# silencht/SG-SLAM

Measured on AMD Instinct MI355X. Metric: tracked frames/sec (640x480 RGB-D), higher is better.
Workload: dtype u8/f32(bf16x3 matrix products)/f64

## Files before the change

include/sgx_debug.h:

```cpp
#ifndef SGX_DEBUG_H
#define SGX_DEBUG_H
#include "sgx.h"
#ifdef __cplusplus
extern "C" {
#endif

int sgx_orb_debug_level_geometry(const sgx_orb *h, int level, int32_t *w, int32_t *hgt, int32_t *stride);
int sgx_orb_debug_set_unfused_pyramid(int on);
int sgx_orb_debug_read_level(sgx_orb *h, int frame, int level, uint8_t *dst );
int sgx_orb_debug_read_candidates(sgx_orb *h, int frame, int level, int32_t *x, int32_t *y, int32_t *score, int cap, int *n);
int sgx_debug_flow_affine_batch_dev(int batch, int cap, const sgx_keypoint *d_keys, const int32_t *d_n, const float *d_A, const float *d_shift, const float *d_boxes,
                                    int max_boxes, float *d_prev_xy, void *stream);
int sgx_pose_opt_debug_set_threads(int threads_per_frame);
int sgx_ba_debug_last_plan(int32_t plan[4]);
int sgx_ba_debug_set_init(int mode);
int sgx_ba_debug_set_jobs(int host);
int sgx_ba_debug_set_solver(int mode);
int sgx_det_debug_read_blob(sgx_det *h, const char *blob_name, int image, float *dst, int cap, int *n);
int sgx_flow_debug_read_level(sgx_flow *h, int slot, int frame, int level, uint8_t *img);
int sgx_flow_debug_read_slot(sgx_flow *h, int slot, int frame, int level, uint8_t *img, int32_t *pitch);
int sgx_flow_debug_level_size(const sgx_flow *h, int level, int32_t *w, int32_t *hgt);
int sgx_pnp_debug_betas(int which, const double *L, const double *rho, double *betas);
int sgx_obj3d_debug_read(sgx_obj3d *h, int job, uint8_t *kept, int32_t *labels, int cap, int *n);
int sgx_cloud_debug_read(sgx_cloud *h, int image, sgx_cloud_point *voxels, float *dist, uint8_t *kept, int cap, int *n);
int sgx_debug_corun_bf16(int blocks, int iters, int launches, void *stream);
int sgx_det_debug_detection_output(sgx_det *h, const float *loc, const float *conf, int batch, sgx_det_result *results);
int sgx_det_debug_continued(sgx_det *h, int *count);
int sgx_det_debug_set_fusion(int on);
int sgx_det_debug_set_irb(int on);
int sgx_det_debug_set_block_fusion(int on);
int sgx_det_debug_set_gemm(int mode);
int sgx_det_debug_set_legacy_kernels(int on);
int sgx_det_debug_time_ops(sgx_det *h, const uint8_t *d_img, int pitch, int batch, int reps, float *ms, int cap, int *nops);
int sgx_det_debug_run_step(sgx_det *h, const uint8_t *d_img, int pitch, int batch, int step, int reps, void *stream);
int sgx_orb_debug_run_octree(sgx_orb *h, int level, const uint32_t *packed, int n, uint32_t *out_sel, int cap, int *nsel);
int sgx_orb_debug_read_plan(const sgx_orb *h, int section, void *dst, size_t cap, size_t *bytes);
int sgx_tracker_debug_set_describe_early(int on);
int sgx_tracker_debug_set_boxes(sgx_tracker *t, const float *boxes, const int32_t *nboxes, const int32_t *have_dynamic);
int sgx_tracker_debug_sync_trace(sgx_tracker *t, int32_t *dst, int cap, int *n);
int sgx_tracker_debug_fail_after(int n);
int sgx_debug_devmem_fail_after(int n);
int sgx_stereo_debug_read(sgx_stereo *h, int frame, int32_t *best_idx, int32_t *best_dist, int32_t *exit_code, int32_t *best_inc, int32_t *sads);

#ifdef __cplusplus
}
#endif
#endif
```

sg_slam_amd/capi.py:

```python
import ctypes as C
import numpy as np

KP_DTYPE = np.dtype([('x', 'f4'), ('y', 'f4'), ('size', 'f4'), ('angle', 'f4'), ('response', 'f4'),
                     ('octave', 'i4'), ('class_id', 'i4')])


class SgxError(RuntimeError):
    pass


class Camera(C.Structure):
    _fields_ = [('fx', C.c_float), ('fy', C.c_float), ('cx', C.c_float), ('cy', C.c_float), ('bf', C.c_float),
                ('min_x', C.c_float), ('max_x', C.c_float), ('min_y', C.c_float), ('max_y', C.c_float)]


class BaProblem(C.Structure):
    _fields_ = [('n_poses', C.c_int32), ('n_points', C.c_int32), ('n_edges', C.c_int32), ('poses', C.c_void_p), ('pose_fixed', C.c_void_p),
                ('points', C.c_void_p), ('edge_pose', C.c_void_p), ('edge_point', C.c_void_p), ('edge_obs', C.c_void_p), ('edge_info', C.c_void_p)]


class BaStats(C.Structure):
    _fields_ = [('iterations_first', C.c_int32), ('iterations_second', C.c_int32), ('free_poses', C.c_int32), ('reserved', C.c_int32),
                ('chi2_first', C.c_double), ('chi2_second', C.c_double)]


SGX_DET_MAX = 100


class Detection(C.Structure):
    _fields_ = [(k, C.c_float) for k in ('label', 'score', 'xmin', 'ymin', 'xmax', 'ymax')]


class Object2D(C.Structure):
    _fields_ = [('id', C.c_int32)] + [(k, C.c_float) for k in ('prob', 'x', 'y', 'w', 'h')]


class DetResult(C.Structure):
    _fields_ = [('n_raw', C.c_int32), ('raw', Detection * SGX_DET_MAX), ('n_objects', C.c_int32), ('objects', Object2D * SGX_DET_MAX),
                ('have_dynamic_for_mapping', C.c_int32), ('have_dynamic_for_rm_feature', C.c_int32),
                ('n_map_boxes', C.c_int32), ('map_boxes', Object2D * SGX_DET_MAX), ('n_rm_boxes', C.c_int32), ('rm_boxes', Object2D * SGX_DET_MAX)]


class FlowConfig(C.Structure):
    _fields_ = [('width', C.c_int32), ('height', C.c_int32), ('max_batch', C.c_int32), ('win_size', C.c_int32), ('max_level', C.c_int32),
                ('max_count', C.c_int32), ('epsilon', C.c_double)]


class TrackerConfig(C.Structure):
    _fields_ = [('streams', C.c_int32), ('width', C.c_int32), ('height', C.c_int32), ('nfeatures', C.c_int32), ('scale_factor', C.c_float), ('nlevels', C.c_int32),
                ('ini_th_fast', C.c_int32), ('min_th_fast', C.c_int32), ('cam', Camera), ('depth_map_factor', C.c_float), ('th_projection', C.c_float),
                ('local_map', C.c_int32), ('dynamic_mask', C.c_int32), ('max_boxes', C.c_int32), ('pipelined', C.c_int32)]


class Obj3dParams(C.Structure):
    _fields_ = [('sor_stddev_mul', C.c_double), ('sor_mean_k', C.c_int32), ('cluster_min_size', C.c_int32), ('cluster_max_size', C.c_int32),
                ('voxel_leaf_size', C.c_float), ('cluster_tolerance', C.c_float), ('similar_compare_ratio', C.c_float),
                ('camera_valid_depth_min', C.c_float), ('camera_valid_depth_max', C.c_float)]


class Obj3dJob(C.Structure):
    _fields_ = [('image', C.c_int32), ('class_id', C.c_int32)] + [(k, C.c_float) for k in ('prob', 'x', 'y', 'w', 'h')]


OBJ3D_RESULT_DTYPE = np.dtype([('found', 'i4'), ('class_id', 'i4'), ('prob', 'f4'), ('centroid', 'f4', 3), ('size', 'f4', 3), ('crop_points', 'i4'), ('kept_points', 'i4'),
                               ('components', 'i4'), ('clusters', 'i4'), ('best_cluster_size', 'i4'), ('larger_window_points', 'i4'), ('best_similar1', 'f4'),
                               ('best_similar2', 'f4'), ('best_roi', 'f4', 4)])


class SemanticObjectRecord(C.Structure):
    _fields_ = [('class_id', C.c_int32), ('object_id', C.c_int32), ('prob', C.c_float), ('centroid', C.c_float * 3), ('size', C.c_float * 3)]


class CloudParams(C.Structure):
    _fields_ = [('sor_stddev_mul', C.c_double), ('sor_mean_k', C.c_int32), ('consider_dynamic', C.c_int32), ('voxel_leaf_size', C.c_float),
                ('camera_valid_depth_min', C.c_float), ('camera_valid_depth_max', C.c_float), ('reserved', C.c_int32)]


CLOUD_POINT_DTYPE = np.dtype([('x', 'f4'), ('y', 'f4'), ('z', 'f4'), ('rgba', 'u4')])
CLOUD_RESULT_DTYPE = np.dtype([('n_points', 'i4'), ('n_pixels_used', 'i4'), ('n_voxels', 'i4'), ('flags', 'i4'), ('larger_window_points', 'i4'), ('reserved', 'i4'),
                               ('mean', 'f8'), ('thr', 'f8')])
SGX_CLOUD_LOCAL, SGX_CLOUD_WORLD = 0, 1
SGX_CLOUD_FEW_POINTS, SGX_CLOUD_LEAF_TOO_SMALL = 1, 2
SGX_CLOUD_MAX_BOXES = 128


class InitReport(C.Structure):
    _fields_ = [('SH', C.c_float), ('SF', C.c_float), ('RH', C.c_float), ('model', C.c_int32), ('n_matches', C.c_int32), ('n_inliers_h', C.c_int32),
                ('n_inliers_f', C.c_int32), ('n_hyp', C.c_int32), ('best_hyp', C.c_int32), ('n_good', C.c_int32 * 8), ('cos_parallax', C.c_float * 8),
                ('parallax', C.c_float * 8), ('H21', C.c_float * 9), ('F21', C.c_float * 9)]


class KfdbReport(C.Structure):
    _fields_ = [('n_sharing', C.c_int32), ('max_common_words', C.c_int32), ('min_common_words', C.c_int32), ('n_scores', C.c_int32), ('n_score_and_match', C.c_int32),
                ('best_acc_score', C.c_float), ('min_score_to_retain', C.c_float), ('n_candidates', C.c_int32), ('status', C.c_int32)]


KFDB_REPORT_DTYPE = np.dtype([('n_sharing', 'i4'), ('max_common_words', 'i4'), ('min_common_words', 'i4'), ('n_scores', 'i4'), ('n_score_and_match', 'i4'),
                              ('best_acc_score', 'f4'), ('min_score_to_retain', 'f4'), ('n_candidates', 'i4'), ('status', 'i4')])


class OrbConfig(C.Structure):
    _fields_ = [('nfeatures', C.c_int32), ('scale_factor', C.c_float), ('nlevels', C.c_int32),
                ('ini_th_fast', C.c_int32), ('min_th_fast', C.c_int32), ('width', C.c_int32),
                ('height', C.c_int32), ('max_batch', C.c_int32)]


SYMBOLS = [
    'sgx_version', 'sgx_status_string', 'sgx_orb_create', 'sgx_orb_destroy', 'sgx_orb_keypoint_capacity', 'sgx_orb_get_tables',
    'sgx_orb_extract_batch_dev', 'sgx_orb_extract', 'sgx_orb_last_status', 'sgx_profile_enable', 'sgx_profile_num_classes', 'sgx_profile_class_name',
    'sgx_profile_read', 'sgx_match_project_frame_batch_dev', 'sgx_match_project_frame', 'sgx_match_project_local_batch_dev',
    'sgx_match_project_local', 'sgx_frame_stereo_from_rgbd_batch_dev', 'sgx_frame_unproject_batch_dev', 'sgx_frame_make_map_points_batch_dev',
    'sgx_frame_merge_matches_batch_dev', 'sgx_pose_optimization_batch_dev', 'sgx_pose_optimization', 'sgx_frame_motion_model_batch_dev',
    'sgx_local_bundle_adjustment', 'sgx_bundle_adjustment', 'sgx_det_create', 'sgx_det_destroy', 'sgx_det_info', 'sgx_det_detect',
    'sgx_det_detect_batch_dev', 'sgx_det_forward_batch_dev', 'sgx_frame_compact_keys_batch_dev', 'sgx_frame_gray_from_color_batch_dev',
    'sgx_det_gemm_mode', 'sgx_det_plan_step', 'sgx_dynamic_mask_batch_dev', 'sgx_tracker_create', 'sgx_tracker_destroy',
    'sgx_tracker_keypoint_capacity', 'sgx_tracker_record_bytes', 'sgx_tracker_set_initial_pose', 'sgx_tracker_step_dev', 'sgx_tracker_host_buffers',
    'sgx_tracker_step_host', 'sgx_tracker_wait_inputs', 'sgx_tracker_sync', 'sgx_tracker_read', 'sgx_tracker_snapshot_pose_dev',
    'sgx_tracker_snapshot_boxes_dev', 'sgx_tracker_pack_records_dev', 'sgx_tracker_frame_dev', 'sgx_tracker_extractor', 'sgx_flow_create',
    'sgx_dist_unique_id', 'sgx_dist_create', 'sgx_dist_destroy', 'sgx_dist_world', 'sgx_dist_gather_records',
    'sgx_flow_destroy', 'sgx_flow_reset', 'sgx_flow_levels', 'sgx_flow_lk_batch_dev', 'sgx_flow_lk', 'sgx_fundamental_ransac_batch_dev',
    'sgx_find_fundamental_mat', 'sgx_hamming_matrix', 'sgx_hamming_matrix_dev', 'sgx_match_search_for_triangulation', 'sgx_match_search_by_bow',
    'sgx_match_search_by_bow_kf', 'sgx_match_fuse_search', 'sgx_match_project_keyframe', 'sgx_match_fuse_search_sim3',
    'sgx_triangulate_new_map_points', 'sgx_mappoint_update_normal_and_depth', 'sgx_mappoint_distinctive_descriptors', 'sgx_sim3_solver_create',
    'sgx_sim3_solver_set_ransac_parameters', 'sgx_sim3_solver_iterate', 'sgx_sim3_solver_get_estimate', 'sgx_sim3_solver_destroy',
    'sgx_match_search_for_initialization', 'sgx_voc_load', 'sgx_voc_create', 'sgx_voc_info', 'sgx_voc_destroy', 'sgx_voc_transform',
    'sgx_voc_transform_batch_dev', 'sgx_voc_score', 'sgx_match_project_sim3', 'sgx_match_search_by_sim3', 'sgx_optimize_sim3',
    'sgx_optimize_essential_graph', 'sgx_correct_map_points', 'sgx_undistort_points', 'sgx_frame_undistort_stereo_rgbd_batch_dev', 'sgx_frame_image_bounds',
    'sgx_tracker_set_distortion', 'sgx_tracker_frame_keys_un_dev', 'sgx_pnp_solver_create', 'sgx_pnp_solver_set_ransac_parameters', 'sgx_pnp_solver_iterate',
    'sgx_pnp_solver_get_estimate', 'sgx_pnp_solver_destroy', 'sgx_pnp_batch_create', 'sgx_pnp_batch_set_dev', 'sgx_pnp_batch_iterate_dev', 'sgx_pnp_batch_destroy',
    'sgx_obj3d_create', 'sgx_obj3d_destroy', 'sgx_obj3d_detect_batch_dev', 'sgx_obj3d_detect', 'sgx_objdb_create', 'sgx_objdb_destroy', 'sgx_objdb_add', 'sgx_objdb_size',
    'sgx_objdb_get', 'sgx_initializer_create', 'sgx_initializer_initialize', 'sgx_initializer_destroy', 'sgx_init_batch_create', 'sgx_init_batch_run_dev',
    'sgx_init_batch_destroy', 'sgx_orb_detect_batch_dev', 'sgx_orb_describe_batch_dev', 'sgx_frame_compact_keys_src_batch_dev',
    'sgx_voc_bow_batch_dev', 'sgx_kfdb_create', 'sgx_kfdb_destroy', 'sgx_kfdb_size', 'sgx_kfdb_add', 'sgx_kfdb_erase', 'sgx_kfdb_clear', 'sgx_kfdb_set_covisibility',
    'sgx_kfdb_slots', 'sgx_kfdb_detect_relocalization_candidates', 'sgx_kfdb_detect_loop_candidates', 'sgx_kfdb_min_score', 'sgx_kfdb_detect_batch_dev',
    'sgx_cloud_create', 'sgx_cloud_destroy', 'sgx_cloud_build_batch_dev', 'sgx_cloud_build', 'sgx_cloud_camera_to_map_tf',
    'sgx_stereo_create', 'sgx_stereo_destroy', 'sgx_stereo_match_batch_dev', 'sgx_stereo_match',
]
TAP_SYMBOLS = [
    'sgx_orb_debug_level_geometry', 'sgx_orb_debug_set_unfused_pyramid', 'sgx_orb_debug_read_level', 'sgx_orb_debug_read_candidates',
    'sgx_orb_debug_run_octree', 'sgx_orb_debug_read_plan', 'sgx_pose_opt_debug_set_threads', 'sgx_ba_debug_set_solver', 'sgx_ba_debug_set_jobs', 'sgx_ba_debug_set_init', 'sgx_ba_debug_last_plan', 'sgx_det_debug_read_blob',
    'sgx_det_debug_detection_output', 'sgx_det_debug_continued', 'sgx_debug_flow_affine_batch_dev', 'sgx_det_debug_set_fusion', 'sgx_det_debug_set_legacy_kernels',
    'sgx_det_debug_set_block_fusion', 'sgx_det_debug_set_irb', 'sgx_det_debug_set_gemm', 'sgx_det_debug_time_ops', 'sgx_det_debug_run_step', 'sgx_flow_debug_read_level',
    'sgx_flow_debug_level_size', 'sgx_flow_debug_read_slot', 'sgx_debug_corun_bf16', 'sgx_pnp_debug_betas', 'sgx_obj3d_debug_read',
    'sgx_tracker_debug_set_describe_early', 'sgx_tracker_debug_set_boxes', 'sgx_tracker_debug_sync_trace', 'sgx_tracker_debug_fail_after',
    'sgx_debug_devmem_fail_after', 'sgx_cloud_debug_read', 'sgx_stereo_debug_read',
]


def _vp(x):
    if x is None:
        return None
    if isinstance(x, int):
        return C.c_void_p(x)
    if hasattr(x, 'data_ptr'):
        return C.c_void_p(x.data_ptr())
    return x.ctypes.data_as(C.c_void_p)


class SgxLib:
    def __init__(self, path):
        self.path = path
        self.dll = C.CDLL(path)
        d = self.dll
        d.sgx_version.restype = C.c_char_p
        d.sgx_status_string.restype = C.c_char_p
        d.sgx_status_string.argtypes = [C.c_int]
        d.sgx_orb_create.argtypes = [C.POINTER(OrbConfig), C.POINTER(C.c_void_p)]
        d.sgx_orb_destroy.argtypes = [C.c_void_p]
        d.sgx_orb_destroy.restype = None
        d.sgx_orb_keypoint_capacity.argtypes = [C.c_void_p]
        d.sgx_orb_get_tables.argtypes = [C.c_void_p] + [C.c_void_p] * 5
        d.sgx_orb_extract_batch_dev.argtypes = [C.c_void_p, C.c_void_p, C.c_int, C.c_int, C.c_void_p, C.c_void_p,
                                                C.c_void_p, C.c_int, C.c_void_p]
        d.sgx_orb_detect_batch_dev.argtypes = [C.c_void_p, C.c_void_p, C.c_int, C.c_int, C.c_void_p, C.c_void_p, C.c_int, C.c_void_p]
        d.sgx_orb_describe_batch_dev.argtypes = [C.c_void_p, C.c_void_p, C.c_int, C.c_int, C.c_void_p, C.c_void_p, C.c_void_p, C.c_void_p, C.c_int, C.c_void_p]
        d.sgx_orb_extract.argtypes = [C.c_void_p, C.c_void_p, C.c_int, C.c_void_p, C.c_void_p, C.c_int, C.POINTER(C.c_int)]
        d.sgx_orb_last_status.argtypes = [C.c_void_p, C.c_void_p]

        d.sgx_profile_enable.argtypes = [C.c_int]
        d.sgx_profile_class_name.restype = C.c_char_p
        d.sgx_profile_class_name.argtypes = [C.c_int]
        d.sgx_profile_read.argtypes = [C.c_void_p, C.c_void_p, C.c_int]

        vp = C.c_void_p
        d.sgx_match_project_frame_batch_dev.argtypes = [C.c_int, C.c_int] + [vp] * 13 + [C.POINTER(Camera), vp, C.c_int, C.c_float, C.c_int, C.c_int, vp, vp, vp]
        d.sgx_match_project_frame.argtypes = [C.c_int] + [vp] * 4 + [C.c_int] + [vp] * 7 + [C.POINTER(Camera), vp, C.c_int, C.c_float, C.c_int, C.c_int, vp, vp]
        d.sgx_frame_stereo_from_rgbd_batch_dev.argtypes = [C.c_int, C.c_int, vp, vp, vp, C.c_int, C.c_int, C.c_float, C.c_float, vp, vp, vp]
        d.sgx_frame_unproject_batch_dev.argtypes = [C.c_int, C.c_int, vp, vp, vp, vp, C.POINTER(Camera), vp, vp, vp]
        d.sgx_pose_optimization_batch_dev.argtypes = [C.c_int, C.c_int, vp, vp, vp, vp, vp, vp, C.c_int, vp, C.c_int, C.POINTER(Camera), vp, vp, vp, vp]
        d.sgx_pose_optimization.argtypes = [C.c_int, vp, vp, vp, vp, vp, C.c_int, C.POINTER(Camera), vp, vp, vp]
        d.sgx_frame_motion_model_batch_dev.argtypes = [C.c_int, vp, vp, vp, vp, vp]
        d.sgx_local_bundle_adjustment.argtypes = [C.POINTER(BaProblem), C.POINTER(Camera), vp, vp, C.POINTER(BaStats)]
        d.sgx_bundle_adjustment.argtypes = [C.POINTER(BaProblem), C.POINTER(Camera), C.c_int, vp, C.c_int, C.POINTER(BaStats)]
        d.sgx_det_create.argtypes = [C.c_char_p, vp, C.c_size_t, C.c_int, C.c_int, C.c_int, C.c_float, C.c_float, C.POINTER(vp)]
        d.sgx_det_destroy.argtypes = [vp]; d.sgx_det_destroy.restype = None
        d.sgx_det_info.argtypes = [vp, C.POINTER(C.c_int32), C.POINTER(C.c_int32), C.POINTER(C.c_int32), C.POINTER(C.c_double)]
        d.sgx_det_detect.argtypes = [vp, vp, C.c_int, C.c_int, C.POINTER(DetResult)]
        d.sgx_det_detect_batch_dev.argtypes = [vp, vp, C.c_int, C.c_int, vp, vp, vp, C.c_int, vp, vp]
        d.sgx_det_forward_batch_dev.argtypes = [vp, vp, C.c_int, C.c_int, C.POINTER(vp), C.POINTER(vp), vp]
        d.sgx_det_gemm_mode.argtypes = [vp]
        d.sgx_tracker_create.argtypes = [C.POINTER(TrackerConfig), vp, C.POINTER(vp)]
        d.sgx_tracker_destroy.argtypes = [vp]; d.sgx_tracker_destroy.restype = None
        d.sgx_tracker_keypoint_capacity.argtypes = [vp]
        d.sgx_tracker_record_bytes.argtypes = [vp]
        d.sgx_tracker_set_initial_pose.argtypes = [vp, vp]
        d.sgx_tracker_step_dev.argtypes = [vp, vp, C.c_int, vp, vp, C.c_int, vp]
        d.sgx_tracker_host_buffers.argtypes = [vp, C.c_int, C.POINTER(vp), C.POINTER(C.c_int), C.POINTER(vp)]
        d.sgx_tracker_step_host.argtypes = [vp, C.c_int, C.c_int]
        d.sgx_tracker_sync.argtypes = [vp]
        d.sgx_tracker_wait_inputs.argtypes = [vp, C.c_int]
        d.sgx_tracker_read.argtypes = [vp] * 10
        d.sgx_tracker_snapshot_pose_dev.argtypes = [vp, vp]
        d.sgx_tracker_snapshot_boxes_dev.argtypes = [vp, C.c_int, vp, vp]
        d.sgx_tracker_pack_records_dev.argtypes = [vp, vp, vp]
        d.sgx_dist_unique_id.argtypes = [vp]
        d.sgx_dist_create.argtypes = [vp, C.c_int, C.c_int, C.POINTER(vp)]
        d.sgx_dist_destroy.argtypes = [vp]; d.sgx_dist_destroy.restype = None
        d.sgx_dist_world.argtypes = [vp, C.POINTER(C.c_int32), C.POINTER(C.c_int32)]
        d.sgx_dist_gather_records.argtypes = [vp, vp, C.c_size_t, vp, C.c_int, vp]
        d.sgx_tracker_frame_dev.argtypes = [vp] + [C.POINTER(vp)] * 6
        d.sgx_tracker_extractor.argtypes = [vp]; d.sgx_tracker_extractor.restype = vp
        d.sgx_det_plan_step.argtypes = [vp, C.c_int, C.c_char_p, C.c_int]
        d.sgx_dynamic_mask_batch_dev.argtypes = [C.c_int, C.c_int, vp, vp, vp, vp, vp, vp, C.c_int, vp, vp]
        d.sgx_frame_gray_from_color_batch_dev.argtypes = [C.c_int, C.c_int, C.c_int, vp, C.c_int, C.c_int, C.c_int, vp, C.c_int, vp]
        d.sgx_frame_compact_keys_batch_dev.argtypes = [C.c_int, C.c_int, vp, vp, vp, vp, vp, C.c_int, vp, vp, vp, vp]
        d.sgx_frame_compact_keys_src_batch_dev.argtypes = [C.c_int, C.c_int, vp, vp, vp, vp, C.c_int, vp, vp, vp, vp]
        d.sgx_match_project_local.argtypes = [C.c_int] + [vp] * 5 + [C.c_int] + [vp] * 7 + [C.POINTER(Camera), vp, C.c_int, C.c_float, C.c_float, C.c_float, C.c_float, vp, vp, vp]
        d.sgx_match_project_local_batch_dev.argtypes = [C.c_int, C.c_int] + [vp] * 6 + [C.c_int] + [vp] * 8 + [C.POINTER(Camera), vp, C.c_int, C.c_float, C.c_float, C.c_float, C.c_float, vp, vp, vp, vp]
        d.sgx_undistort_points.argtypes = [C.c_int, vp, vp, vp, C.c_int, vp]
        d.sgx_frame_undistort_stereo_rgbd_batch_dev.argtypes = [C.c_int, C.c_int, vp, vp, vp, C.c_int, C.POINTER(Camera), vp, C.c_int, C.c_int, C.c_float, vp, vp, vp, vp]
        d.sgx_frame_image_bounds.argtypes = [C.c_int, C.c_int, vp, vp, C.c_int, C.POINTER(Camera)]
        d.sgx_tracker_set_distortion.argtypes = [vp, vp, C.c_int, C.POINTER(Camera)]
        d.sgx_tracker_frame_keys_un_dev.argtypes = [vp, C.POINTER(vp)]
        d.sgx_frame_make_map_points_batch_dev.argtypes = [C.c_int, C.c_int, C.c_int] + [vp] * 7 + [C.c_int] + [vp] * 7
        d.sgx_frame_merge_matches_batch_dev.argtypes = [C.c_int, C.c_int] + [vp] * 10
        d.sgx_flow_create.argtypes = [C.POINTER(FlowConfig), C.POINTER(vp)]
        d.sgx_flow_destroy.argtypes = [vp]; d.sgx_flow_destroy.restype = None
        d.sgx_flow_reset.argtypes = [vp]
        d.sgx_flow_levels.argtypes = [vp]
        d.sgx_flow_lk_batch_dev.argtypes = [vp, vp, C.c_int, C.c_int, vp, vp, C.c_int, vp, vp, C.POINTER(C.c_int32), vp]
        d.sgx_flow_lk.argtypes = [vp, vp, vp, C.c_int, vp, C.c_int, vp, vp]
        d.sgx_fundamental_ransac_batch_dev.argtypes = [C.c_int, C.c_int] + [vp] * 6 + [C.c_int, C.c_double, C.c_double, vp, vp, vp, vp]
        d.sgx_find_fundamental_mat.argtypes = [vp, vp, C.c_int, C.c_double, C.c_double, vp, vp, vp]
        d.sgx_hamming_matrix.argtypes = [vp, C.c_int, vp, C.c_int, vp]
        d.sgx_optimize_essential_graph.argtypes = [C.c_int, vp, vp, C.c_int, vp, vp, vp, C.c_int, C.c_int, vp, vp]
        d.sgx_correct_map_points.argtypes = [C.c_int, vp, vp, C.c_int, vp, vp, vp]
        d.sgx_optimize_sim3.argtypes = [C.c_int] + [vp] * 9 + [C.c_float, C.c_int, vp, vp, vp]
        d.sgx_match_project_keyframe.argtypes = [C.c_int] + [vp] * 4 + [C.c_int] + [vp] * 6 + [C.POINTER(Camera), vp, C.c_int, C.c_float, C.c_float, C.c_int, C.c_int, vp, vp]
        d.sgx_match_search_by_bow.argtypes = [C.c_int] + [vp] * 4 + [C.c_int] + [vp] * 3 + [C.c_float, C.c_int, vp, vp]
        d.sgx_match_fuse_search_sim3.argtypes = [C.c_int, vp, vp, vp, C.c_int] + [vp] * 6 + [vp, vp, C.c_int, C.c_float, C.c_float, vp, vp, vp]
        d.sgx_match_project_sim3.argtypes = [C.c_int, vp, vp, vp, vp, C.c_int] + [vp] * 6 + [vp, vp, C.c_int, C.c_float, C.c_int, vp, vp]
        d.sgx_match_search_by_sim3.argtypes = ([C.c_int] + [vp] * 8) * 2 + [vp, vp, C.c_int, C.c_float, C.c_float, vp, vp, C.c_float, vp, vp]
        d.sgx_match_search_for_initialization.argtypes = [C.c_int, vp, vp, C.c_int, vp, vp, vp, C.c_int, C.c_float, C.c_int, vp, vp, vp]
        d.sgx_sim3_solver_create.argtypes = [C.c_int] + [vp] * 6 + [C.c_int, C.c_uint, vp]
        d.sgx_sim3_solver_set_ransac_parameters.argtypes = [vp, C.c_double, C.c_int, C.c_int]
        d.sgx_sim3_solver_iterate.argtypes = [vp, C.c_int] + [vp] * 7
        d.sgx_sim3_solver_get_estimate.argtypes = [vp] * 5
        d.sgx_sim3_solver_destroy.argtypes = [vp]; d.sgx_sim3_solver_destroy.restype = None
        d.sgx_pnp_solver_create.argtypes = [C.c_int] + [vp] * 4 + [C.c_uint, vp]
        d.sgx_pnp_solver_set_ransac_parameters.argtypes = [vp, C.c_double, C.c_int, C.c_int, C.c_int, C.c_float, C.c_float]
        d.sgx_pnp_solver_iterate.argtypes = [vp, C.c_int] + [vp] * 7
        d.sgx_pnp_solver_get_estimate.argtypes = [vp] * 6
        d.sgx_pnp_solver_destroy.argtypes = [vp]; d.sgx_pnp_solver_destroy.restype = None
        d.sgx_pnp_batch_create.argtypes = [C.c_int, C.c_int, vp]
        d.sgx_pnp_batch_set_dev.argtypes = [vp, C.c_int] + [vp] * 8
        d.sgx_pnp_batch_iterate_dev.argtypes = [vp, C.c_int, vp, C.c_int, vp, vp, vp, vp]
        d.sgx_pnp_batch_destroy.argtypes = [vp]; d.sgx_pnp_batch_destroy.restype = None
        d.sgx_initializer_create.argtypes = [C.c_int, vp, vp, C.c_float, C.c_int, C.c_uint, vp]
        d.sgx_initializer_initialize.argtypes = [vp, C.c_int] + [vp] * 10
        d.sgx_initializer_destroy.argtypes = [vp]; d.sgx_initializer_destroy.restype = None
        d.sgx_init_batch_create.argtypes = [C.c_int] * 4 + [vp]
        d.sgx_init_batch_run_dev.argtypes = [vp, C.c_int] + [vp] * 9 + [C.c_int] + [vp] * 8
        d.sgx_init_batch_destroy.argtypes = [vp]; d.sgx_init_batch_destroy.restype = None
        d.sgx_obj3d_create.argtypes = [C.c_int] * 5 + [C.POINTER(Obj3dParams), C.POINTER(vp)]
        d.sgx_obj3d_destroy.argtypes = [vp]; d.sgx_obj3d_destroy.restype = None
        d.sgx_obj3d_detect_batch_dev.argtypes = [vp, vp, C.c_int, C.c_int, vp, vp, vp, C.c_int, vp, vp]
        d.sgx_obj3d_detect.argtypes = [vp, vp, vp, vp, C.POINTER(Obj3dJob), vp]
        d.sgx_objdb_create.argtypes = [C.POINTER(vp)]
        d.sgx_objdb_destroy.argtypes = [vp]; d.sgx_objdb_destroy.restype = None
        d.sgx_objdb_add.argtypes = [vp, C.POINTER(SemanticObjectRecord), C.POINTER(C.c_int32), C.POINTER(C.c_int32)]
        d.sgx_objdb_size.argtypes = [vp]
        d.sgx_objdb_get.argtypes = [vp, C.c_int, C.POINTER(SemanticObjectRecord)]
        d.sgx_cloud_create.argtypes = [C.c_int] * 5 + [C.POINTER(CloudParams), C.POINTER(vp)]
        d.sgx_cloud_destroy.argtypes = [vp]; d.sgx_cloud_destroy.restype = None
        d.sgx_cloud_build_batch_dev.argtypes = [vp, vp, C.c_int, vp, C.c_int, C.c_int] + [vp] * 8
        d.sgx_cloud_build.argtypes = [vp] * 6 + [C.c_int, C.c_int, vp, C.c_int, vp]
        d.sgx_cloud_camera_to_map_tf.argtypes = [vp, vp, vp]
        d.sgx_stereo_create.argtypes = [vp, C.c_int, C.POINTER(vp)]
        d.sgx_stereo_destroy.argtypes = [vp]; d.sgx_stereo_destroy.restype = None
        d.sgx_stereo_match_batch_dev.argtypes = [vp, C.c_int] + [vp, C.c_int, vp, C.c_int] * 2 + [C.c_int] + [vp] * 6 + [C.c_float, C.c_float, vp, vp, vp, vp]
        d.sgx_stereo_match.argtypes = [vp, vp, vp, vp, vp, C.c_int, vp, vp, C.c_int, C.c_float, C.c_float, vp, vp, vp]
        d.sgx_mappoint_update_normal_and_depth.argtypes = [C.c_int] + [vp] * 6 + [C.c_int, vp, vp, vp]
        d.sgx_mappoint_distinctive_descriptors.argtypes = [C.c_int, vp, vp, vp, vp]
        d.sgx_triangulate_new_map_points.argtypes = [C.c_int, vp] + [C.c_int] + [vp] * 5 + [C.c_int] + [vp] * 5 + [vp, vp, vp, C.c_int, vp, vp, vp]
        d.sgx_voc_load.argtypes = [C.c_char_p, vp]
        d.sgx_voc_create.argtypes = [C.c_int] * 5 + [vp] * 5
        d.sgx_voc_info.argtypes = [vp] * 7
        d.sgx_voc_destroy.argtypes = [vp]; d.sgx_voc_destroy.restype = None
        d.sgx_voc_transform.argtypes = [vp, C.c_int, vp, C.c_int, vp, vp, vp, vp, vp]
        d.sgx_voc_transform_batch_dev.argtypes = [vp, vp, C.c_size_t, vp, C.c_int, C.c_int, C.c_int, vp, vp, vp, vp]
        d.sgx_voc_score.argtypes = [vp, C.c_int, vp, vp, C.c_int, vp, vp, vp]
        d.sgx_voc_bow_batch_dev.argtypes = [vp, vp, C.c_int, C.c_int] + [vp] * 6
        d.sgx_kfdb_create.argtypes = [vp] + [C.c_int] * 4 + [vp]
        d.sgx_kfdb_destroy.argtypes = [vp]; d.sgx_kfdb_destroy.restype = None
        d.sgx_kfdb_size.argtypes = [vp]
        d.sgx_kfdb_add.argtypes = [vp, C.c_int32, C.c_int, vp, vp]
        d.sgx_kfdb_erase.argtypes = [vp, C.c_int32]
        d.sgx_kfdb_clear.argtypes = [vp]
        d.sgx_kfdb_set_covisibility.argtypes = [vp, C.c_int32, C.c_int, vp]
        d.sgx_kfdb_slots.argtypes = [vp, vp, vp]
        d.sgx_kfdb_detect_relocalization_candidates.argtypes = [vp, C.c_int, vp, vp, vp, vp, C.POINTER(KfdbReport)]
        d.sgx_kfdb_detect_loop_candidates.argtypes = [vp, C.c_int, vp, vp, C.c_int, vp, C.c_float, vp, vp, C.POINTER(KfdbReport)]
        d.sgx_kfdb_min_score.argtypes = [vp, C.c_int, vp, vp, C.c_int, vp, vp]
        d.sgx_kfdb_detect_batch_dev.argtypes = [vp, C.c_int, C.c_int, vp, vp, C.c_int] + [vp] * 10
        d.sgx_match_search_by_bow_kf.argtypes = [C.c_int] + [vp] * 4 + [C.c_int] + [vp] * 4 + [C.c_float, C.c_int, vp, vp]
        d.sgx_match_fuse_search.argtypes = [C.c_int] + [vp] * 4 + [C.c_int] + [vp] * 6 + [C.POINTER(Camera), vp, vp, C.c_int, C.c_float, C.c_float, vp, vp, vp]
        d.sgx_hamming_matrix_dev.argtypes = [vp, C.c_int, vp, C.c_int, vp, vp]
        d.sgx_match_search_for_triangulation.argtypes = [C.c_int] + [vp] * 6 + [C.c_int] + [vp] * 6 + [vp, C.POINTER(Camera), vp, vp, C.c_int, C.c_int, C.c_int, vp, vp]

        self.has_taps = hasattr(d, 'sgx_det_debug_read_blob')
        if self.has_taps:
            d.sgx_orb_debug_level_geometry.argtypes = [C.c_void_p, C.c_int] + [C.POINTER(C.c_int32)] * 3
            d.sgx_orb_debug_read_level.argtypes = [C.c_void_p, C.c_int, C.c_int, C.c_void_p]
            d.sgx_orb_debug_read_candidates.argtypes = [C.c_void_p, C.c_int, C.c_int, C.c_void_p, C.c_void_p, C.c_void_p, C.c_int, C.POINTER(C.c_int)]
            d.sgx_orb_debug_run_octree.argtypes = [C.c_void_p, C.c_int, C.c_void_p, C.c_int, C.c_void_p, C.c_int, C.POINTER(C.c_int)]
            d.sgx_orb_debug_set_unfused_pyramid.argtypes = [C.c_int]
            if hasattr(d, 'sgx_orb_debug_read_plan'):
                d.sgx_orb_debug_read_plan.argtypes = [C.c_void_p, C.c_int, C.c_void_p, C.c_size_t, C.POINTER(C.c_size_t)]
            d.sgx_pose_opt_debug_set_threads.argtypes = [C.c_int]
            d.sgx_ba_debug_set_solver.argtypes = [C.c_int]
            d.sgx_ba_debug_set_jobs.argtypes = [C.c_int]
            d.sgx_ba_debug_set_init.argtypes = [C.c_int]
            d.sgx_ba_debug_last_plan.argtypes = [C.c_void_p]
            d.sgx_det_debug_detection_output.argtypes = [vp, vp, vp, C.c_int, C.POINTER(DetResult)]
            d.sgx_det_debug_continued.argtypes = [vp, C.POINTER(C.c_int)]
            d.sgx_det_debug_read_blob.argtypes = [vp, C.c_char_p, C.c_int, vp, C.c_int, C.POINTER(C.c_int)]
            for nm in ('fusion', 'legacy_kernels', 'block_fusion', 'irb', 'gemm'):
                getattr(d, 'sgx_det_debug_set_' + nm).argtypes = [C.c_int]
            d.sgx_det_debug_time_ops.argtypes = [vp, vp, C.c_int, C.c_int, C.c_int, vp, C.c_int, C.POINTER(C.c_int)]
            d.sgx_det_debug_run_step.argtypes = [vp, vp, C.c_int, C.c_int, C.c_int, C.c_int, vp]
            d.sgx_debug_flow_affine_batch_dev.argtypes = [C.c_int, C.c_int, vp, vp, vp, vp, vp, C.c_int, vp, vp]
            d.sgx_flow_debug_read_level.argtypes = [vp, C.c_int, C.c_int, C.c_int, vp]
            d.sgx_debug_corun_bf16.argtypes = [C.c_int, C.c_int, C.c_int, vp]
            d.sgx_pnp_debug_betas.argtypes = [C.c_int, vp, vp, vp]
            d.sgx_obj3d_debug_read.argtypes = [vp, C.c_int, vp, vp, C.c_int, C.POINTER(C.c_int)]
            d.sgx_flow_debug_level_size.argtypes = [vp, C.c_int, C.POINTER(C.c_int32), C.POINTER(C.c_int32)]
            d.sgx_flow_debug_read_slot.argtypes = [vp, C.c_int, C.c_int, C.c_int, vp, C.POINTER(C.c_int32)]
            d.sgx_tracker_debug_set_describe_early.argtypes = [C.c_int]
            d.sgx_tracker_debug_set_boxes.argtypes = [vp, vp, vp, vp]
            if hasattr(d, 'sgx_tracker_debug_sync_trace'):
                d.sgx_tracker_debug_sync_trace.argtypes = [vp, vp, C.c_int, C.POINTER(C.c_int)]
            if hasattr(d, 'sgx_tracker_debug_fail_after'):
                d.sgx_tracker_debug_fail_after.argtypes = [C.c_int]
            if hasattr(d, 'sgx_debug_devmem_fail_after'):
                d.sgx_debug_devmem_fail_after.argtypes = [C.c_int]
            if hasattr(d, 'sgx_cloud_debug_read'):
                d.sgx_cloud_debug_read.argtypes = [vp, C.c_int, vp, vp, vp, C.c_int, C.POINTER(C.c_int)]
            if hasattr(d, 'sgx_stereo_debug_read'):
                d.sgx_stereo_debug_read.argtypes = [vp, C.c_int, vp, vp, vp, vp, vp]

    def tap(self, name):
        if not self.has_taps:
            raise SgxError(f'{name}: {self.path} is the product build and has no test taps; use tests/taps/libsgx_taps.so (make -C sg_slam_amd/csrc taps)')
        return getattr(self.dll, name)

    def version(self):
        return self.dll.sgx_version().decode()

    def check(self, rc, what=''):
        if rc != 0:
            raise SgxError(f'{what}: {self.dll.sgx_status_string(rc).decode()} ({rc})')

    def profile_enable(self, on=True):
        self.check(self.dll.sgx_profile_enable(int(on)))

    def profile_read(self, reset=True):
        n = self.dll.sgx_profile_num_classes()
        ms = np.zeros(n, 'f4'); cnt = np.zeros(n, 'i4')
        self.check(self.dll.sgx_profile_read(_vp(ms), _vp(cnt), int(reset)), 'sgx_profile_read')
        return {self.dll.sgx_profile_class_name(k).decode(): (float(ms[k]), int(cnt[k])) for k in range(n)}
```

sg_slam_amd/csrc/sgx_block.h:

```cpp
#pragma once
#include "sgx_rt.h"

#ifdef SGX_EMU
SGX_DEV void sgx_block_exclusive_scan_i32(int *a, int n, int *total, int tid)
{
    if (tid != 0) return;
    int run = 0;
    for (int i = 0; i < n; i++) { const int v = a[i]; a[i] = run; run += v; }
    *total = run;
}
#else
SGX_DEV void sgx_block_exclusive_scan_i32(int *a, int n, int *total, int tid)
{
    if (tid >= 64) return;
    int carry = 0;
    for (int base = 0; base < n; base += 64) {
        const int i = base + tid;
        const int v = i < n ? a[i] : 0;
        int inc = v;
#pragma unroll
        for (int o = 1; o < 64; o <<= 1) { const int t = __shfl_up(inc, o, 64); if (tid >= o) inc += t; }
        if (i < n) a[i] = carry + inc - v;
        carry += __shfl(inc, 63, 64);
    }
    if (tid == 0) *total = carry;
}
#endif
```

sg_slam_amd/csrc/sgx_match.cpp:

```cpp
#include "sgx_match_kernels.h"
#include "sgx_host_args.h"
#include "sgx_prof.h"
#include "sgx_stage.h"
#include "../../include/sgx.h"
#ifdef SGX_DEBUG_TAPS
#include "../../include/sgx_debug.h"
#endif
#include <stdio.h>
#include <stdlib.h>
#include <string.h>
#include <vector>


extern "C" int sgx_match_project_frame_batch_dev(
    int batch, int cap,
    const sgx_keypoint *d_ckeys, const uint8_t *d_cdesc, const float *d_curight, const int32_t *d_cn, const float *d_cTcw,
    const sgx_keypoint *d_lkeys, const int32_t *d_ln, const uint8_t *d_l_has_mp, const uint8_t *d_l_outlier, const float *d_l_xw,
    const int32_t *d_l_obs, const uint8_t *d_l_mpdesc, const float *d_lTcw,
    const sgx_camera *cam, const float *scale_factors, int nlevels, float th, int b_mono, int check_orientation,
    int32_t *d_cur_match, int32_t *d_nmatches, void *stream)
{
    if (batch < 1 || cap < 1 || cap > SGX_MATCH_CAP || !cam || !scale_factors || nlevels < 1 || nlevels > 12) return SGX_ERR_INVALID;
    if (!d_ckeys || !d_cdesc || !d_curight || !d_cn || !d_cTcw || !d_lkeys || !d_ln || !d_l_has_mp || !d_l_outlier || !d_l_xw ||
        !d_l_obs || !d_l_mpdesc || !d_lTcw || !d_cur_match || !d_nmatches) return SGX_ERR_INVALID;
    const SgxScales sc = to_scales(scale_factors, nlevels);
    sgx_prof_begin(SGX_K_MATCH, (sgx_stream_t)stream);
    static const int mthreads = sgx_getenv("SGX_TUNE_MATCH_THREADS") ? atoi(sgx_getenv("SGX_TUNE_MATCH_THREADS")) : SGX_MATCH_THREADS;
    SGX_LAUNCH(k_match_project_frame, dim3(batch), dim3(mthreads), (sgx_stream_t)stream, cap,
               (const uint8_t *)d_ckeys, d_cdesc, d_curight, d_cn, d_cTcw, (const uint8_t *)d_lkeys, d_ln, d_l_has_mp, d_l_outlier,
               d_l_xw, d_l_obs, d_l_mpdesc, d_lTcw, to_cam(cam), sc, th, b_mono, check_orientation, d_cur_match, d_nmatches);
    sgx_prof_end(SGX_K_MATCH, (sgx_stream_t)stream);
    SGX_CHECK_HIP(hipGetLastError());
    return SGX_OK;
}

extern "C" int sgx_frame_stereo_from_rgbd_batch_dev(int batch, int cap, const sgx_keypoint *d_keys, const int32_t *d_n,
                                                     const uint16_t *d_depth, int width, int height, float depth_map_factor,
                                                     float bf, float *d_uright, float *d_zdepth, void *stream)
{
    if (batch < 1 || cap < 1 || !d_keys || !d_n || !d_depth || !d_uright || !d_zdepth || !(depth_map_factor > 0)) return SGX_ERR_INVALID;
    const float inv = 1.0f / depth_map_factor;
    sgx_prof_begin(SGX_K_STEREO, (sgx_stream_t)stream);
    SGX_LAUNCH(k_stereo_from_rgbd, dim3((cap + 255) / 256, batch), dim3(256), (sgx_stream_t)stream, cap, (const uint8_t *)d_keys, d_n,
               d_depth, width, height, inv, bf, d_uright, d_zdepth);
    sgx_prof_end(SGX_K_STEREO, (sgx_stream_t)stream);
    SGX_CHECK_HIP(hipGetLastError());
    return SGX_OK;
}

extern "C" int sgx_frame_unproject_batch_dev(int batch, int cap, const sgx_keypoint *d_keys, const int32_t *d_n, const float *d_zdepth,
                                              const float *d_Tcw, const sgx_camera *cam, float *d_xw, uint8_t *d_has, void *stream)
{
    if (batch < 1 || cap < 1 || !d_keys || !d_n || !d_zdepth || !d_Tcw || !cam || !d_xw || !d_has) return SGX_ERR_INVALID;
    sgx_prof_begin(SGX_K_UNPROJECT, (sgx_stream_t)stream);
    SGX_LAUNCH(k_unproject, dim3((cap + 255) / 256, batch), dim3(256), (sgx_stream_t)stream, cap, (const uint8_t *)d_keys, d_n, d_zdepth,
               d_Tcw, to_cam(cam), d_xw, d_has);
    sgx_prof_end(SGX_K_UNPROJECT, (sgx_stream_t)stream);
    SGX_CHECK_HIP(hipGetLastError());
    return SGX_OK;
}

extern "C" int sgx_match_project_local_batch_dev(
    int batch, int cap, const sgx_keypoint *d_ckeys, const uint8_t *d_cdesc, const float *d_curight, const int32_t *d_cn, const float *d_cTcw, const int32_t *d_cur_mp_obs,
    int mcap, const int32_t *d_mn, const float *d_m_xw, const float *d_m_normal, const float *d_m_min_dist, const float *d_m_max_dist, const uint8_t *d_m_desc,
    const int32_t *d_m_obs, const uint8_t *d_m_skip,
    const sgx_camera *cam, const float *scale_factors, int nlevels, float log_scale_factor, float th, float nnratio, float viewing_cos_limit,
    int32_t *d_cur_match, int32_t *d_nmatches, uint8_t *d_in_view, void *stream)
{
    if (batch < 1 || cap < 1 || cap > SGX_MATCH_CAP || mcap < 1 || mcap > SGX_LOCAL_CAP || !cam || !scale_factors || nlevels < 1 || nlevels > 12) return SGX_ERR_INVALID;
    if (!d_ckeys || !d_cdesc || !d_curight || !d_cn || !d_cTcw || !d_mn || !d_m_xw || !d_m_normal || !d_m_min_dist || !d_m_max_dist || !d_m_desc || !d_m_obs ||
        !d_m_skip || !d_cur_match || !d_nmatches || !d_in_view) return SGX_ERR_INVALID;
    const SgxScales sc = to_scales(scale_factors, nlevels);
    sgx_prof_begin(SGX_K_MATCH_LOCAL, (sgx_stream_t)stream);
    SGX_LAUNCH(k_match_project_local, dim3(batch), dim3(SGX_MATCH_THREADS), (sgx_stream_t)stream, cap, (const uint8_t *)d_ckeys, d_cdesc, d_curight, d_cn, d_cTcw,
               d_cur_mp_obs, mcap, d_mn, d_m_xw, d_m_normal, d_m_min_dist, d_m_max_dist, d_m_desc, d_m_obs, d_m_skip, to_cam(cam), sc, nlevels, log_scale_factor,
               th, nnratio, viewing_cos_limit, d_cur_match, d_nmatches, d_in_view);
    sgx_prof_end(SGX_K_MATCH_LOCAL, (sgx_stream_t)stream);
    SGX_CHECK_HIP(hipGetLastError());
    return SGX_OK;
}

extern "C" int sgx_frame_make_map_points_batch_dev(int batch, int cap, int half, const sgx_keypoint *d_keys, const int32_t *d_n, const float *d_xw, const uint8_t *d_has,
                                                    const uint8_t *d_desc, const float *d_Tcw, const float *scale_factors, int nlevels,
                                                    float *d_m_xw, float *d_m_normal, float *d_m_min_dist, float *d_m_max_dist, uint8_t *d_m_desc, uint8_t *d_m_skip, void *stream)
{
    if (batch < 1 || cap < 1 || half < 0 || half > 1 || !d_keys || !d_n || !d_xw || !d_has || !d_desc || !d_Tcw || !scale_factors || nlevels < 1 || nlevels > 12 ||
        !d_m_xw || !d_m_normal || !d_m_min_dist || !d_m_max_dist || !d_m_desc || !d_m_skip) return SGX_ERR_INVALID;
    const SgxScales sc = to_scales(scale_factors, nlevels);
    sgx_prof_begin(SGX_K_MAPGLUE, (sgx_stream_t)stream);
    SGX_LAUNCH(k_make_map_points, dim3((cap + 255) / 256, batch), dim3(256), (sgx_stream_t)stream, cap, half, (const uint8_t *)d_keys, d_n, d_xw, d_has, d_desc, d_Tcw, sc, nlevels,
               d_m_xw, d_m_normal, d_m_min_dist, d_m_max_dist, d_m_desc, d_m_skip);
    sgx_prof_end(SGX_K_MAPGLUE, (sgx_stream_t)stream);
    SGX_CHECK_HIP(hipGetLastError());
    return SGX_OK;
}

extern "C" int sgx_frame_merge_matches_batch_dev(int batch, int cap, const int32_t *d_n, const int32_t *d_match_last, const uint8_t *d_outlier_last, const int32_t *d_match_local,
                                                  const float *d_xw_last, const float *d_m_xw, int32_t *d_merged, int32_t *d_cur_mp_obs, float *d_xw_all, void *stream)
{
    if (batch < 1 || cap < 1 || !d_n || !d_match_last || !d_outlier_last) return SGX_ERR_INVALID;
    sgx_prof_begin(SGX_K_MAPGLUE, (sgx_stream_t)stream);
    SGX_LAUNCH(k_merge_matches, dim3((cap + 255) / 256, batch), dim3(256), (sgx_stream_t)stream, cap, d_n, d_match_last, d_outlier_last, d_match_local, d_merged, d_cur_mp_obs);
    if (d_xw_all && d_xw_last && d_m_xw)
        SGX_LAUNCH(k_gather_xw, dim3((3 * cap + 255) / 256, batch), dim3(256), (sgx_stream_t)stream, cap, d_xw_last, d_m_xw, d_xw_all);
    sgx_prof_end(SGX_K_MAPGLUE, (sgx_stream_t)stream);
    SGX_CHECK_HIP(hipGetLastError());
    return SGX_OK;
}

extern "C" int sgx_frame_motion_model_batch_dev(int batch, const float *d_Tcw_cur, const float *d_Tcw_prev, const uint8_t *d_valid, float *d_Tcw_pred, void *stream)
{
    if (batch < 1 || !d_Tcw_cur || !d_Tcw_prev || !d_Tcw_pred) return SGX_ERR_INVALID;
    sgx_prof_begin(SGX_K_MOTION, (sgx_stream_t)stream);
    SGX_LAUNCH(k_motion_model, dim3((batch + 63) / 64), dim3(64), (sgx_stream_t)stream, batch, d_Tcw_cur, d_Tcw_prev, d_valid, d_Tcw_pred);
    sgx_prof_end(SGX_K_MOTION, (sgx_stream_t)stream);
    SGX_CHECK_HIP(hipGetLastError());
    return SGX_OK;
}

extern "C" int sgx_match_project_frame(
    int nc, const sgx_keypoint *ckeys, const uint8_t *cdesc, const float *curight, const float *cTcw,
    int nl, const sgx_keypoint *lkeys, const uint8_t *l_has_mp, const uint8_t *l_outlier, const float *l_xw,
    const int32_t *l_obs, const uint8_t *l_mpdesc, const float *lTcw,
    const sgx_camera *cam, const float *scale_factors, int nlevels, float th, int b_mono, int check_orientation,
    int32_t *cur_match, int32_t *nmatches)
{
    if (nc < 0 || nl < 0 || nc > SGX_MATCH_CAP || nl > SGX_MATCH_CAP || !cur_match || !nmatches || !cTcw || !lTcw || !cam || !scale_factors || nlevels < 1) return SGX_ERR_INVALID;
    if (nc > 0 && (!ckeys || !cdesc || !curight)) return SGX_ERR_INVALID;
    if (nl > 0 && (!lkeys || !l_has_mp || !l_outlier || !l_xw || !l_obs || !l_mpdesc)) return SGX_ERR_INVALID;
    int cap = nc > nl ? nc : nl; if (cap < 1) cap = 1;
    SgxStaging st(SGX_STAGE_FRAME_MATCH);
    std::vector<uint8_t> pad;
    auto padded = [&](auto *src, int per, int n) {
        const size_t elem = (size_t)per * sizeof *src;
        pad.assign((size_t)cap * elem, 0);
        if (n > 0 && src) memcpy(pad.data(), src, (size_t)n * elem);
        const uint8_t *d = st.in(pad.data(), pad.size());
        if (st.rc == SGX_OK) st.hip(hipStreamSynchronize(0));
        return (decltype(src))d;
    };
    const sgx_keypoint *d_ckeys = padded(ckeys, 1, nc); const uint8_t *d_cdesc = padded(cdesc, 32, nc); const float *d_curight = padded(curight, 1, nc);
    const sgx_keypoint *d_lkeys = padded(lkeys, 1, nl); const uint8_t *d_has = padded(l_has_mp, 1, nl), *d_outlier = padded(l_outlier, 1, nl);
    const float *d_lxw = padded(l_xw, 3, nl); const int32_t *d_lobs = padded(l_obs, 1, nl); const uint8_t *d_mpdesc = padded(l_mpdesc, 32, nl);
    const int32_t *d_nc = st.in(&nc, 1), *d_nl = st.in(&nl, 1);
    const float *d_cTcw = st.in(cTcw, 16), *d_lTcw = st.in(lTcw, 16);
    int32_t *d_match = st.out<int32_t>(cap), *d_nmatches = st.out<int32_t>(1);
    if (st.rc != SGX_OK) return st.rc;
    SGX_CHECK_HIP(hipStreamSynchronize(0));
    const int rc = sgx_match_project_frame_batch_dev(1, cap, d_ckeys, d_cdesc, d_curight, d_nc, d_cTcw, d_lkeys, d_nl, d_has, d_outlier, d_lxw, d_lobs, d_mpdesc, d_lTcw,
                                                     cam, scale_factors, nlevels, th, b_mono, check_orientation, d_match, d_nmatches, nullptr);
    if (rc != SGX_OK) return rc;
    st.back(cur_match, d_match, nc); st.back(nmatches, d_nmatches, 1);
    return st.rc;
}

extern "C" int sgx_match_project_local(
    int nc, const sgx_keypoint *ckeys, const uint8_t *cdesc, const float *curight, const float *cTcw, const int32_t *cur_mp_obs,
    int nm, const float *m_xw, const float *m_normal, const float *m_min_dist, const float *m_max_dist, const uint8_t *m_desc, const int32_t *m_obs, const uint8_t *m_skip,
    const sgx_camera *cam, const float *scale_factors, int nlevels, float log_scale_factor, float th, float nnratio, float viewing_cos_limit,
    int32_t *cur_match, int32_t *nmatches, uint8_t *in_view)
{
    if (nc < 0 || nm < 0 || nc > SGX_MATCH_CAP || nm > SGX_LOCAL_CAP || !cur_match || !nmatches || !cTcw || !cam || !scale_factors) return SGX_ERR_INVALID;
    for (int i = 0; i < nc; i++) cur_match[i] = -1;
    if (in_view) memset(in_view, 0, (size_t)nm);
    *nmatches = 0;
    if (nc == 0 || nm == 0) return SGX_OK;
    std::vector<int32_t> no_obs;
    if (!cur_mp_obs) { no_obs.assign((size_t)nc, -1); cur_mp_obs = no_obs.data(); }
    SgxStaging st(SGX_STAGE_LOCAL_MATCH);
    const sgx_keypoint *d_ckeys = st.in(ckeys, nc); const uint8_t *d_cdesc = st.in(cdesc, (size_t)nc * 32); const float *d_curight = st.in(curight, nc);
    const int32_t *d_nc = st.in(&nc, 1); const float *d_cTcw = st.in(cTcw, 16); const int32_t *d_obs = st.in(cur_mp_obs, nc);
    const int32_t *d_nm = st.in(&nm, 1); const float *d_xw = st.in(m_xw, (size_t)nm * 3), *d_normal = st.in(m_normal, (size_t)nm * 3);
    const float *d_min = st.in(m_min_dist, nm), *d_max = st.in(m_max_dist, nm);
    const uint8_t *d_mdesc = st.in(m_desc, (size_t)nm * 32); const int32_t *d_mobs = st.in(m_obs, nm); const uint8_t *d_skip = st.in(m_skip, nm);
    int32_t *d_match = st.out<int32_t>(nc), *d_nmatches = st.out<int32_t>(1); uint8_t *d_in_view = st.out<uint8_t>(nm);
    if (st.rc != SGX_OK) return st.rc;
    SGX_CHECK_HIP(hipStreamSynchronize(0));
    const int rc = sgx_match_project_local_batch_dev(1, nc, d_ckeys, d_cdesc, d_curight, d_nc, d_cTcw, d_obs, nm, d_nm, d_xw, d_normal, d_min, d_max, d_mdesc, d_mobs, d_skip,
                                                     cam, scale_factors, nlevels, log_scale_factor, th, nnratio, viewing_cos_limit, d_match, d_nmatches, d_in_view, nullptr);
    if (rc != SGX_OK) return rc;
    st.back(cur_match, d_match, nc); st.back(nmatches, d_nmatches, 1);
    if (in_view) st.back(in_view, d_in_view, nm);
    return st.rc;
}

extern "C" int sgx_frame_gray_from_color_batch_dev(int batch, int width, int height, const uint8_t *d_src, int src_pitch, int channels, int blue_first,
                                                   uint8_t *d_gray, int gray_pitch, void *stream)
{
    if (batch < 1 || width < 1 || height < 1 || !d_src || !d_gray || (channels != 3 && channels != 4) || src_pitch < width * channels || gray_pitch < width ||
        (src_pitch & 3) || (gray_pitch & 3) || ((uintptr_t)d_src & 3) || ((uintptr_t)d_gray & 3)) return SGX_ERR_INVALID;
    SGX_LAUNCH(k_gray_from_color, dim3((width + 255) / 256, height, batch), dim3(64), (sgx_stream_t)stream, width, height, d_src, src_pitch, channels, blue_first ? 1 : 0, d_gray, gray_pitch);
    SGX_CHECK_HIP(hipGetLastError());
    return SGX_OK;
}

SGX_TAP int sgx_debug_flow_affine_batch_dev(int batch, int cap, const sgx_keypoint *d_keys, const int32_t *d_n, const float *d_A, const float *d_shift, const float *d_boxes,
                                               int max_boxes, float *d_prev_xy, void *stream)
{
    if (batch < 1 || cap < 1 || !d_keys || !d_n || !d_A || !d_prev_xy) return SGX_ERR_INVALID;
    SGX_LAUNCH(k_flow_affine, dim3((cap + 255) / 256, batch), dim3(256), (sgx_stream_t)stream, cap, (const uint8_t *)d_keys, d_n, d_A, d_shift, d_boxes, max_boxes, d_prev_xy);
    SGX_CHECK_HIP(hipGetLastError());
    return SGX_OK;
}
```

sg_slam_amd/csrc/sgx_match_kernels.h:

```cpp
#pragma once
#include "sgx_rt.h"

#define SGX_GRID_COLS 64
#define SGX_GRID_ROWS 48
#define SGX_MATCH_CAP 1280
#define SGX_MATCH_THREADS 1024

#include "sgx_match_common.h"


SGX_KERNEL(SGX_MATCH_THREADS) k_match_project_frame(
    int cap, const uint8_t *ckeys_raw, const uint8_t *cdesc, const float *curight, const int *cn, const float *cTcw,
    const uint8_t *lkeys_raw, const int *ln, const uint8_t *l_has_mp, const uint8_t *l_outlier, const float *l_xw,
    const int *l_obs, const uint8_t *l_mpdesc, const float *lTcw,
    SgxCam cam, SgxScales sc, float th, int bMono, int check_ori, int *cur_match, int *nmatches_out)
{
    SGX_LDS float kx[SGX_MATCH_CAP], ky[SGX_MATCH_CAP], kur[SGX_MATCH_CAP], kang[SGX_MATCH_CAP];
    SGX_LDS uint32_t kinfo[SGX_MATCH_CAP];
    SGX_LDS uint32_t kdesc[SGX_MATCH_CAP * 8];
    SGX_LDS int lock_a[SGX_MATCH_CAP], lock_b[SGX_MATCH_CAP];
    SGX_LDS int choice[SGX_MATCH_CAP];
    SGX_LDS int owner[SGX_MATCH_CAP];
    SGX_LDS int hist[SGX_HISTO], bad[SGX_HISTO];
    SGX_LDS int cell_start[SGX_GRID_COLS * SGX_GRID_ROWS + 1];
    SGX_LDS int cell_fill[SGX_GRID_COLS * SGX_GRID_ROWS];
    SGX_LDS uint16_t cell_list[SGX_MATCH_CAP];
    SGX_LDS int s_changed, s_total, s_rejected, s_ngrid;

    const int f = (int)blockIdx.x;
    SGX_WAVE_PRIORITY(3);
    const int Nc = min(cn[f], cap), Nl = min(ln[f], cap);
    const int NT = (int)blockDim.x;
    const float *Tc = cTcw + 16 * f, *Tl = lTcw + 16 * f;
    const float invW = (float)SGX_GRID_COLS / (cam.maxX - cam.minX), invH = (float)SGX_GRID_ROWS / (cam.maxY - cam.minY);

    SGX_THREADS_BEGIN(tid)
    for (int k = tid; k < Nc; k += NT) {
        const float *kp = (const float *)(ckeys_raw + ((size_t)f * cap + k) * 28);
        const float x = kp[0], y = kp[1];
        kx[k] = x; ky[k] = y; kang[k] = kp[3]; kur[k] = curight[(size_t)f * cap + k];
        const int oct = ((const int *)kp)[5];
        const int px = (int)round((double)((x - cam.minX) * invW)), py = (int)round((double)((y - cam.minY) * invH));
        const bool valid = !(px < 0 || px >= SGX_GRID_COLS || py < 0 || py >= SGX_GRID_ROWS);
        kinfo[k] = (uint32_t)(oct & 0xFF) | ((uint32_t)(px & 0xFF) << 8) | ((uint32_t)(py & 0xFF) << 16) | (valid ? 0x80000000u : 0u);
        const uint32_t *d = (const uint32_t *)(cdesc + ((size_t)f * cap + k) * 32);
#pragma unroll
        for (int w = 0; w < 8; w++) kdesc[k * 8 + w] = d[w];
        lock_a[k] = 0x7FFFFFFF; owner[k] = -1;
    }
    for (int i = tid; i < SGX_HISTO; i += NT) { hist[i] = 0; bad[i] = 0; }
    for (int i = tid; i < SGX_GRID_COLS * SGX_GRID_ROWS; i += NT) { cell_start[i] = 0; cell_fill[i] = 0; }
    if (tid == 0) { s_total = 0; s_rejected = 0; }
    SGX_THREADS_END
    SGX_SYNC();
    SGX_THREADS_BEGIN(tid)
    for (int k = tid; k < Nc; k += NT) { const uint32_t inf = kinfo[k]; if (inf & 0x80000000u) sgx_atomic_add(&cell_start[((inf >> 8) & 0xFF) * SGX_GRID_ROWS + ((inf >> 16) & 0xFF)], 1); }
    SGX_THREADS_END
    SGX_SYNC();
    SGX_THREADS_BEGIN(tid)
    sgx_block_exclusive_scan_i32(cell_start, SGX_GRID_COLS * SGX_GRID_ROWS, &s_ngrid, tid);
    SGX_THREADS_END
    SGX_SYNC();
    SGX_THREADS_BEGIN(tid)
    if (tid == 0) cell_start[SGX_GRID_COLS * SGX_GRID_ROWS] = s_ngrid;
    for (int k = tid; k < Nc; k += NT) {
        const uint32_t inf = kinfo[k];
        if (inf & 0x80000000u) { const int c = ((inf >> 8) & 0xFF) * SGX_GRID_ROWS + ((inf >> 16) & 0xFF); cell_list[cell_start[c] + sgx_atomic_add(&cell_fill[c], 1)] = (uint16_t)k; }
    }
    SGX_THREADS_END
    SGX_SYNC();

    float Rcw[3][3], tcw[3];
    for (int r = 0; r < 3; r++) { for (int c = 0; c < 3; c++) Rcw[r][c] = Tc[4 * r + c]; tcw[r] = Tc[4 * r + 3]; }
    float twc[3];
    for (int i = 0; i < 3; i++) {
        double s = 0; for (int k = 0; k < 3; k++) s += (double)Rcw[k][i] * (double)tcw[k];
        twc[i] = (float)(s * -1.0);
    }
    const float Rl2[3] = { Tl[8], Tl[9], Tl[10] };
    const float tlc2 = sgx_gemm3(Rl2, twc, Tl[11]);
    const float mb = cam.bf / cam.fx;
    const bool bForward = tlc2 > mb && !bMono, bBackward = -tlc2 > mb && !bMono;

    int *lock_cur = lock_a, *lock_new = lock_b;
    for (int sweep = 0; sweep < SGX_MATCH_CAP + 2; sweep++) {
        SGX_THREADS_BEGIN(tid)
        if (tid == 0) s_changed = 0;
        for (int k = tid; k < Nc; k += NT) lock_new[k] = 0x7FFFFFFF;
        SGX_THREADS_END
        SGX_SYNC();
        SGX_THREADS_BEGIN(tid)
        for (int i = tid; i < Nl; i += NT) {
            int best = -1;
            const size_t li = (size_t)f * cap + i;
            if (l_has_mp[li] && !l_outlier[li]) {
                const float *xw = l_xw + 3 * li;
                const float x3x = sgx_gemm3(Rcw[0], xw, tcw[0]), x3y = sgx_gemm3(Rcw[1], xw, tcw[1]), x3z = sgx_gemm3(Rcw[2], xw, tcw[2]);
                const float invzc = (float)(1.0 / (double)x3z);
                const float u = cam.fx * x3x * invzc + cam.cx, v = cam.fy * x3y * invzc + cam.cy;
                if (!(invzc < 0) && !(u < cam.minX || u > cam.maxX) && !(v < cam.minY || v > cam.maxY)) {
                    const int lo = ((const int *)(lkeys_raw + li * 28))[5];
                    const float radius = th * sc.s[lo];
                    int minLevel, maxLevel;
                    if (bForward) { minLevel = lo; maxLevel = -1; } else if (bBackward) { minLevel = 0; maxLevel = lo; } else { minLevel = lo - 1; maxLevel = lo + 1; }
                    const int c0x = max(0, (int)floorf((u - cam.minX - radius) * invW)), c1x = min(SGX_GRID_COLS - 1, (int)ceilf((u - cam.minX + radius) * invW));
                    const int c0y = max(0, (int)floorf((v - cam.minY - radius) * invH)), c1y = min(SGX_GRID_ROWS - 1, (int)ceilf((v - cam.minY + radius) * invH));
                    if (!(c0x >= SGX_GRID_COLS || c1x < 0 || c0y >= SGX_GRID_ROWS || c1y < 0)) {
                        const bool chk = (minLevel > 0) || (maxLevel >= 0);
                        const float ur = u - cam.bf * invzc;
                        const uint32_t *dmp = (const uint32_t *)(l_mpdesc + li * 32);
                        uint32_t dm[8];
#pragma unroll
                        for (int w = 0; w < 8; w++) dm[w] = dmp[w];
                        unsigned long long bestKey = ~0ull;
                        for (int px = c0x; px <= c1x; px++)
                        for (int q = cell_start[px * SGX_GRID_ROWS + c0y], qe = cell_start[px * SGX_GRID_ROWS + c1y + 1]; q < qe; q++) {
                            const int k = cell_list[q];
                            const uint32_t inf = kinfo[k];
                            const int oct = inf & 0xFF, py = (inf >> 16) & 0xFF;
                            if (chk) { if (oct < minLevel) continue; if (maxLevel >= 0 && oct > maxLevel) continue; }
                            if (!(fabsf(kx[k] - u) < radius && fabsf(ky[k] - v) < radius)) continue;
                            if (lock_cur[k] < i) continue;
                            if (kur[k] > 0) { if (fabsf(ur - kur[k]) > radius) continue; }
                            const int dist = sgx_hamming256(dm, &kdesc[k * 8]);
                            const unsigned long long key = ((unsigned long long)dist << 28) | ((unsigned long long)px << 22) | ((unsigned long long)py << 16) | (unsigned long long)k;
                            if (key < bestKey) bestKey = key;
                        }
                        if (bestKey != ~0ull && (int)(bestKey >> 28) <= SGX_TH_HIGH) best = (int)(bestKey & 0xFFFF);
                    }
                }
            }
            choice[i] = best;
            if (best >= 0 && l_obs[li] > 0) sgx_atomic_min_i32(&lock_new[best], i);
        }
        SGX_THREADS_END
        SGX_SYNC();
        SGX_THREADS_BEGIN(tid)
        for (int k = tid; k < Nc; k += NT) if (lock_new[k] != lock_cur[k]) s_changed = 1;
        SGX_THREADS_END
        SGX_SYNC();
        int *t = lock_cur; lock_cur = lock_new; lock_new = t;
        if (!s_changed) break;
    }

    SGX_THREADS_BEGIN(tid)
    for (int i = tid; i < Nl; i += NT) {
        const int k = choice[i];
        if (k < 0) continue;
        sgx_atomic_max(&owner[k], i);
        sgx_atomic_add(&s_total, 1);
        if (check_ori) {
            const float la = ((const float *)(lkeys_raw + ((size_t)f * cap + i) * 28))[3];
            float rot = la - kang[k];
            if (rot < 0.0f) rot += 360.0f;
            int bin = (int)round((double)(rot * (SGX_HISTO / 360.0f)));
            if (bin == SGX_HISTO) bin = 0;
            sgx_atomic_add(&hist[bin], 1);
            lock_new[i] = bin;
        }
    }
    SGX_THREADS_END
    SGX_SYNC();
    if (check_ori) {
        SGX_THREADS_BEGIN(tid)
        if (tid == 0) {
            int m1 = 0, m2 = 0, m3 = 0, i1 = -1, i2 = -1, i3 = -1;
            for (int i = 0; i < SGX_HISTO; i++) {
                const int s = hist[i];
                if (s > m1) { m3 = m2; m2 = m1; m1 = s; i3 = i2; i2 = i1; i1 = i; }
                else if (s > m2) { m3 = m2; m2 = s; i3 = i2; i2 = i; }
                else if (s > m3) { m3 = s; i3 = i; }
            }
            if ((float)m2 < 0.1f * (float)m1) { i2 = -1; i3 = -1; }
            else if ((float)m3 < 0.1f * (float)m1) { i3 = -1; }
            for (int i = 0; i < SGX_HISTO; i++) bad[i] = (i != i1 && i != i2 && i != i3);
        }
        SGX_THREADS_END
        SGX_SYNC();
        SGX_THREADS_BEGIN(tid)
        for (int i = tid; i < Nl; i += NT) {
            const int k = choice[i];
            if (k >= 0 && bad[lock_new[i]]) { sgx_atomic_add(&s_rejected, 1); lock_cur[k] = -2; }
        }
        SGX_THREADS_END
        SGX_SYNC();
    }
    SGX_THREADS_BEGIN(tid)
    for (int k = tid; k < Nc; k += NT) cur_match[(size_t)f * cap + k] = (check_ori && lock_cur[k] == -2) ? -1 : owner[k];
    for (int k = Nc + tid; k < cap; k += NT) cur_match[(size_t)f * cap + k] = -1;
    if (tid == 0) nmatches_out[f] = s_total - s_rejected;
    SGX_THREADS_END
}

SGX_KERNEL(256) k_stereo_from_rgbd(int cap, const uint8_t *keys_raw, const int *n, const uint16_t *depth, int W, int H,
                                   float depth_factor_inv, float bf, float *uright, float *zdepth)
{
    SGX_THREADS_BEGIN(tid)
    const int f = (int)blockIdx.y, i = (int)blockIdx.x * 256 + tid;
    if (i < cap) {
        float ur = -1.f, z = -1.f;
        if (i < n[f]) {
            const float *kp = (const float *)(keys_raw + ((size_t)f * cap + i) * 28);
            const int u = (int)kp[0], v = (int)kp[1];
            const float d = (float)depth[((size_t)f * H + v) * W + u] * depth_factor_inv;
            if (d > 0) { z = d; ur = kp[0] - bf / d; }
        }
        uright[(size_t)f * cap + i] = ur; zdepth[(size_t)f * cap + i] = z;
    }
    SGX_THREADS_END
}

SGX_KERNEL(256) k_unproject(int cap, const uint8_t *keys_raw, const int *n, const float *zdepth, const float *Tcw, SgxCam cam,
                            float *xw, uint8_t *has)
{
    SGX_THREADS_BEGIN(tid)
    const int f = (int)blockIdx.y, i = (int)blockIdx.x * 256 + tid;
    if (i < cap) {
        const size_t o = (size_t)f * cap + i;
        uint8_t h = 0;
        float X[3] = {0.f, 0.f, 0.f};
        if (i < n[f]) {
            const float z = zdepth[o];
            if (z > 0) {
                const float *T = Tcw + 16 * f;
                const float *kp = (const float *)(keys_raw + o * 28);
                const float invfx = 1.0f / cam.fx, invfy = 1.0f / cam.fy;
                const float xc[3] = { (kp[0] - cam.cx) * z * invfx, (kp[1] - cam.cy) * z * invfy, z };
                for (int r = 0; r < 3; r++) {
                    double s = 0; for (int k = 0; k < 3; k++) s += (double)T[4 * k + r] * (double)T[4 * k + 3];
                    const float Ow = (float)(s * -1.0);
                    const float Rrow[3] = { T[r], T[4 + r], T[8 + r] };
                    X[r] = sgx_gemm3(Rrow, xc, Ow);
                }
                h = 1;
            }
        }
        xw[3 * o] = X[0]; xw[3 * o + 1] = X[1]; xw[3 * o + 2] = X[2]; has[o] = h;
    }
    SGX_THREADS_END
}

SGX_DEV void sgx_mat4_mul(const float *A, const float *B, float *C)
{
    for (int i = 0; i < 4; i++) for (int j = 0; j < 4; j++) {
        const float t = A[4 * i] * B[j] + A[4 * i + 1] * B[4 + j] + A[4 * i + 2] * B[8 + j] + A[4 * i + 3] * B[12 + j];
        C[4 * i + j] = (float)((double)t * 1.0);
    }
}

SGX_KERNEL(64) k_motion_model(int batch, const float *Tcur, const float *Tprev, const uint8_t *valid, float *Tpred)
{
    SGX_THREADS_BEGIN(tid)
    const int f = (int)blockIdx.x * 64 + tid;
    if (f < batch) {
        const float *Tc = Tcur + 16 * f, *Tp = Tprev + 16 * f;
        float out[16];
        if (valid && !valid[f]) { for (int i = 0; i < 16; i++) out[i] = Tc[i]; }
        else {
            float Twc[16];
            for (int r = 0; r < 3; r++) {
                for (int c = 0; c < 3; c++) Twc[4 * r + c] = Tp[4 * c + r];
                double s = 0; for (int k = 0; k < 3; k++) s += (double)Tp[4 * k + r] * (double)Tp[4 * k + 3];
                Twc[4 * r + 3] = (float)(s * -1.0);
            }
            Twc[12] = 0.f; Twc[13] = 0.f; Twc[14] = 0.f; Twc[15] = 1.f;
            float V[16]; sgx_mat4_mul(Tc, Twc, V);
            sgx_mat4_mul(V, Tc, out);
        }
        for (int i = 0; i < 16; i++) Tpred[16 * f + i] = out[i];
    }
    SGX_THREADS_END
}

#define SGX_LOCAL_CAP 4096
#define SGX_LOCAL_SLOTS (SGX_LOCAL_CAP / SGX_MATCH_THREADS)
#define SGX_LOCAL_KEEP 4

struct SgxLocalProj { float u, v, radius, projXR; int lvl; bool ok; };

SGX_DEV SgxLocalProj sgx_local_project(const float *P, const float *Pn, float max_dist, float min_dist, const float (*Rcw)[3], const float *tcw, const float *Ow,
                                       const SgxCam &cam, const SgxScales &sc, int nlevels, float log_scale_factor, float th, float viewing_cos_limit)
{
    SgxLocalProj r; r.lvl = 0; r.radius = 0.f; r.projXR = 0.f;
    const float pcx = sgx_gemm3(Rcw[0], P, tcw[0]), pcy = sgx_gemm3(Rcw[1], P, tcw[1]), pcz = sgx_gemm3(Rcw[2], P, tcw[2]);
    bool ok = !(pcz < 0.0f);
    const float invz = 1.0f / pcz;
    r.u = cam.fx * pcx * invz + cam.cx; r.v = cam.fy * pcy * invz + cam.cy;
    ok = ok && !(r.u < cam.minX || r.u > cam.maxX) && !(r.v < cam.minY || r.v > cam.maxY);
    const float maxDistance = 1.2f * max_dist, minDistance = 0.8f * min_dist;
    const float po0 = P[0] - Ow[0], po1 = P[1] - Ow[1], po2 = P[2] - Ow[2];
    const float dist = (float)sqrt((double)po0 * po0 + (double)po1 * po1 + (double)po2 * po2);
    ok = ok && !(dist < minDistance || dist > maxDistance);
    const float viewCos = (float)(((double)po0 * Pn[0] + (double)po1 * Pn[1] + (double)po2 * Pn[2]) / (double)dist);
    ok = ok && !(viewCos < viewing_cos_limit);
    r.ok = ok;
    if (ok) {
        int lvl = (int)ceilf((float)log((double)(max_dist / dist)) / log_scale_factor);
        if (lvl < 0) lvl = 0; else if (lvl >= nlevels) lvl = nlevels - 1;
        r.lvl = lvl;
        r.projXR = r.u - cam.bf * invz;
        float rad = viewCos > 0.998 ? 2.5f : 4.0f;
        if (th != 1.0f) rad *= th;
        r.radius = rad * sc.s[lvl];
    }
    return r;
}

#define SGX_LKEY(dd, px, py, k) (((uint32_t)(dd) << 23) | ((uint32_t)(px) << 17) | ((uint32_t)(py) << 11) | (uint32_t)(k))
#define SGX_LKEY_NONE 0xFFFFFFFFu

SGX_KERNEL(SGX_MATCH_THREADS) k_match_project_local(
    int cap, const uint8_t *ckeys_raw, const uint8_t *cdesc, const float *curight, const int *cn, const float *cTcw, const int *cur_mp_obs,
    int mcap, const int *mn, const float *m_xw, const float *m_normal, const float *m_min_dist, const float *m_max_dist, const uint8_t *m_desc,
    const int *m_obs, const uint8_t *m_skip,
    SgxCam cam, SgxScales sc, int nlevels, float log_scale_factor, float th, float nnratio, float viewing_cos_limit,
    int *cur_match, int *nmatches_out, uint8_t *in_view)
{
    SGX_LDS float kx[SGX_MATCH_CAP], ky[SGX_MATCH_CAP], kur[SGX_MATCH_CAP];
    SGX_LDS uint32_t kinfo[SGX_MATCH_CAP];
    SGX_LDS uint32_t kdesc[SGX_MATCH_CAP * 8];
    SGX_LDS int lock_a[SGX_MATCH_CAP], lock_b[SGX_MATCH_CAP];
    SGX_LDS int owner[SGX_MATCH_CAP];
    SGX_LDS int cell_start[SGX_GRID_COLS * SGX_GRID_ROWS + 1];
    SGX_LDS int cell_fill[SGX_GRID_COLS * SGX_GRID_ROWS];
    SGX_LDS uint16_t cell_list[SGX_MATCH_CAP];
    SGX_LDS uint16_t choice[SGX_LOCAL_CAP];
    SGX_LDS int s_changed, s_total, s_ngrid;
    SGX_PRIV_DECL(uint32_t, ckey, SGX_LOCAL_SLOTS * SGX_LOCAL_KEEP, SGX_MATCH_THREADS);
    SGX_PRIV_DECL(uint32_t, cflag, SGX_LOCAL_SLOTS, SGX_MATCH_THREADS);

    const int f = (int)blockIdx.x;
    SGX_WAVE_PRIORITY(3);
    const int Nc = min(cn[f], cap), Nm = min(min(mn[f], mcap), SGX_LOCAL_CAP);
    const int NT = (int)blockDim.x;
    const float *Tc = cTcw + 16 * f;
    const float invW = (float)SGX_GRID_COLS / (cam.maxX - cam.minX), invH = (float)SGX_GRID_ROWS / (cam.maxY - cam.minY);

    SGX_THREADS_BEGIN(tid)
    for (int k = tid; k < Nc; k += NT) {
        const float *kp = (const float *)(ckeys_raw + ((size_t)f * cap + k) * 28);
        const float x = kp[0], y = kp[1];
        kx[k] = x; ky[k] = y; kur[k] = curight[(size_t)f * cap + k];
        const int oct = ((const int *)kp)[5];
        const int px = (int)round((double)((x - cam.minX) * invW)), py = (int)round((double)((y - cam.minY) * invH));
        const bool valid = !(px < 0 || px >= SGX_GRID_COLS || py < 0 || py >= SGX_GRID_ROWS);
        kinfo[k] = (uint32_t)(oct & 0xFF) | ((uint32_t)(px & 0xFF) << 8) | ((uint32_t)(py & 0xFF) << 16) | (valid ? 0x80000000u : 0u);
        const uint32_t *d = (const uint32_t *)(cdesc + ((size_t)f * cap + k) * 32);
#pragma unroll
        for (int w = 0; w < 8; w++) kdesc[k * 8 + w] = d[w];
        lock_a[k] = (cur_mp_obs && cur_mp_obs[(size_t)f * cap + k] > 0) ? -1 : 0x7FFFFFFF;
        owner[k] = -1;
    }
    for (int i = tid; i < SGX_GRID_COLS * SGX_GRID_ROWS; i += NT) { cell_start[i] = 0; cell_fill[i] = 0; }
    if (tid == 0) s_total = 0;
    SGX_THREADS_END
    SGX_SYNC();
    SGX_THREADS_BEGIN(tid)
    for (int k = tid; k < Nc; k += NT) { const uint32_t inf = kinfo[k]; if (inf & 0x80000000u) sgx_atomic_add(&cell_start[((inf >> 8) & 0xFF) * SGX_GRID_ROWS + ((inf >> 16) & 0xFF)], 1); }
    SGX_THREADS_END
    SGX_SYNC();
    SGX_THREADS_BEGIN(tid)
    sgx_block_exclusive_scan_i32(cell_start, SGX_GRID_COLS * SGX_GRID_ROWS, &s_ngrid, tid);
    SGX_THREADS_END
    SGX_SYNC();
    SGX_THREADS_BEGIN(tid)
    if (tid == 0) cell_start[SGX_GRID_COLS * SGX_GRID_ROWS] = s_ngrid;
    for (int k = tid; k < Nc; k += NT) {
        const uint32_t inf = kinfo[k];
        if (inf & 0x80000000u) { const int c = ((inf >> 8) & 0xFF) * SGX_GRID_ROWS + ((inf >> 16) & 0xFF); cell_list[cell_start[c] + sgx_atomic_add(&cell_fill[c], 1)] = (uint16_t)k; }
    }
    SGX_THREADS_END
    SGX_SYNC();

    float Rcw[3][3], tcw[3], Ow[3];
    for (int r = 0; r < 3; r++) { for (int c = 0; c < 3; c++) Rcw[r][c] = Tc[4 * r + c]; tcw[r] = Tc[4 * r + 3]; }
    for (int i = 0; i < 3; i++) { double s = 0; for (int k = 0; k < 3; k++) s += (double)Rcw[k][i] * (double)tcw[k]; Ow[i] = (float)(s * -1.0); }

    SGX_THREADS_BEGIN(tid)
    SGX_PRIV_BIND(ckey, tid); SGX_PRIV_BIND(cflag, tid);
#pragma unroll
    for (int j = 0; j < SGX_LOCAL_SLOTS; j++) {
        const int i = tid + j * SGX_MATCH_THREADS;
        uint32_t c0 = SGX_LKEY_NONE, c1 = SGX_LKEY_NONE, c2 = SGX_LKEY_NONE, c3 = SGX_LKEY_NONE, flag = 0;
        if (i < Nm) {
            const size_t mi = (size_t)f * mcap + i;
            uint8_t vis = 0;
            if (!m_skip[mi]) {
                const SgxLocalProj pr = sgx_local_project(m_xw + 3 * mi, m_normal + 3 * mi, m_max_dist[mi], m_min_dist[mi], Rcw, tcw, Ow, cam, sc, nlevels,
                                                          log_scale_factor, th, viewing_cos_limit);
                if (pr.ok) {
                    vis = 1;
                    if (m_obs[mi] > 0) flag |= 2u;
                    const float u = pr.u, v = pr.v, radius = pr.radius;
                    const int minLevel = pr.lvl - 1, maxLevel = pr.lvl;
                    const int c0x = max(0, (int)floorf((u - cam.minX - radius) * invW)), c1x = min(SGX_GRID_COLS - 1, (int)ceilf((u - cam.minX + radius) * invW));
                    const int c0y = max(0, (int)floorf((v - cam.minY - radius) * invH)), c1y = min(SGX_GRID_ROWS - 1, (int)ceilf((v - cam.minY + radius) * invH));
                    if (!(c0x >= SGX_GRID_COLS || c1x < 0 || c0y >= SGX_GRID_ROWS || c1y < 0)) {
                        const uint32_t *dmp = (const uint32_t *)(m_desc + mi * 32);
                        uint32_t dm[8];
#pragma unroll
                        for (int w = 0; w < 8; w++) dm[w] = dmp[w];
                        int cnt = 0;
                        for (int px = c0x; px <= c1x; px++)
                        for (int q = cell_start[px * SGX_GRID_ROWS + c0y], qe = cell_start[px * SGX_GRID_ROWS + c1y + 1]; q < qe; q++) {
                            const int k = cell_list[q];
                            const uint32_t inf = kinfo[k];
                            const int oct = inf & 0xFF, py = (inf >> 16) & 0xFF;
                            if (oct < minLevel || oct > maxLevel) continue;
                            if (!(fabsf(kx[k] - u) < radius && fabsf(ky[k] - v) < radius)) continue;
                            if (kur[k] > 0) { if (fabsf(pr.projXR - kur[k]) > radius) continue; }
                            const int dd = sgx_hamming256(dm, &kdesc[k * 8]);
                            uint32_t key = SGX_LKEY(dd, px, py, k);
                            cnt++;
                            if (key < c3) {
                                c3 = key;
                                if (c3 < c2) { const uint32_t t = c2; c2 = c3; c3 = t; }
                                if (c2 < c1) { const uint32_t t = c1; c1 = c2; c2 = t; }
                                if (c1 < c0) { const uint32_t t = c0; c0 = c1; c1 = t; }
                            }
                        }
                        if (cnt > SGX_LOCAL_KEEP) flag |= 1u;
                    }
                }
            }
            in_view[mi] = vis;
        }
        ckey[j * SGX_LOCAL_KEEP + 0] = c0; ckey[j * SGX_LOCAL_KEEP + 1] = c1; ckey[j * SGX_LOCAL_KEEP + 2] = c2; ckey[j * SGX_LOCAL_KEEP + 3] = c3;
        cflag[j] = flag;
    }
    SGX_THREADS_END
    SGX_SYNC();

    int *lock_cur = lock_a, *lock_new = lock_b;
    for (int sweep = 0; sweep < SGX_LOCAL_CAP + 2; sweep++) {
        SGX_THREADS_BEGIN(tid)
        if (tid == 0) s_changed = 0;
        for (int k = tid; k < Nc; k += NT) lock_new[k] = (cur_mp_obs && cur_mp_obs[(size_t)f * cap + k] > 0) ? -1 : 0x7FFFFFFF;
        SGX_THREADS_END
        SGX_SYNC();
        SGX_THREADS_BEGIN(tid)
        SGX_PRIV_BIND(ckey, tid); SGX_PRIV_BIND(cflag, tid);
#pragma unroll
        for (int j = 0; j < SGX_LOCAL_SLOTS; j++) {
            const int i = tid + j * SGX_MATCH_THREADS;
            if (i < Nm) {
                uint32_t k1 = SGX_LKEY_NONE, k2 = SGX_LKEY_NONE;
#pragma unroll
                for (int q = 0; q < SGX_LOCAL_KEEP; q++) {
                    const uint32_t key = ckey[j * SGX_LOCAL_KEEP + q];
                    if (key != SGX_LKEY_NONE && !(lock_cur[key & 0x7FF] < i)) { if (k1 == SGX_LKEY_NONE) k1 = key; else if (k2 == SGX_LKEY_NONE) k2 = key; }
                }
                if ((cflag[j] & 1u) && k2 == SGX_LKEY_NONE) {
                    const size_t mi = (size_t)f * mcap + i;
                    const SgxLocalProj pr = sgx_local_project(m_xw + 3 * mi, m_normal + 3 * mi, m_max_dist[mi], m_min_dist[mi], Rcw, tcw, Ow, cam, sc, nlevels,
                                                              log_scale_factor, th, viewing_cos_limit);
                    const float u = pr.u, v = pr.v, radius = pr.radius;
                    const int minLevel = pr.lvl - 1, maxLevel = pr.lvl;
                    const int c0x = max(0, (int)floorf((u - cam.minX - radius) * invW)), c1x = min(SGX_GRID_COLS - 1, (int)ceilf((u - cam.minX + radius) * invW));
                    const int c0y = max(0, (int)floorf((v - cam.minY - radius) * invH)), c1y = min(SGX_GRID_ROWS - 1, (int)ceilf((v - cam.minY + radius) * invH));
                    const uint32_t *dm = (const uint32_t *)(m_desc + mi * 32);
                    k1 = SGX_LKEY_NONE; k2 = SGX_LKEY_NONE;
                    for (int px = c0x; px <= c1x; px++)
                    for (int q = cell_start[px * SGX_GRID_ROWS + c0y], qe = cell_start[px * SGX_GRID_ROWS + c1y + 1]; q < qe; q++) {
                        const int k = cell_list[q];
                        const uint32_t inf = kinfo[k];
                        const int oct = inf & 0xFF, py = (inf >> 16) & 0xFF;
                        if (oct < minLevel || oct > maxLevel) continue;
                        if (!(fabsf(kx[k] - u) < radius && fabsf(ky[k] - v) < radius)) continue;
                        if (lock_cur[k] < i) continue;
                        if (kur[k] > 0) { if (fabsf(pr.projXR - kur[k]) > radius) continue; }
                        const uint32_t key = SGX_LKEY(sgx_hamming256(dm, &kdesc[k * 8]), px, py, k);
                        if (key < k1) { k2 = k1; k1 = key; } else if (key < k2) k2 = key;
                    }
                }
                int best = -1;
                if (k1 != SGX_LKEY_NONE) {
                    const int bestDist = (int)(k1 >> 23), bestLevel = (int)(kinfo[k1 & 0x7FF] & 0xFF);
                    const int bestDist2 = k2 != SGX_LKEY_NONE ? (int)(k2 >> 23) : 256, bestLevel2 = k2 != SGX_LKEY_NONE ? (int)(kinfo[k2 & 0x7FF] & 0xFF) : -1;
                    if (bestDist <= SGX_TH_HIGH && !(bestLevel == bestLevel2 && (float)bestDist > nnratio * (float)bestDist2)) best = (int)(k1 & 0x7FF);
                }
                choice[i] = best >= 0 ? (uint16_t)best : (uint16_t)0xFFFF;
                if (best >= 0 && (cflag[j] & 2u)) sgx_atomic_min_i32(&lock_new[best], i);
            }
        }
        SGX_THREADS_END
        SGX_SYNC();
        SGX_THREADS_BEGIN(tid)
        for (int k = tid; k < Nc; k += NT) if (lock_new[k] != lock_cur[k]) s_changed = 1;
        SGX_THREADS_END
        SGX_SYNC();
        int *t = lock_cur; lock_cur = lock_new; lock_new = t;
        if (!s_changed) break;
    }

    SGX_THREADS_BEGIN(tid)
    for (int i = tid; i < Nm; i += NT) { const int k = choice[i]; if (k != 0xFFFF) { sgx_atomic_max(&owner[k], i); sgx_atomic_add(&s_total, 1); } }
    SGX_THREADS_END
    SGX_SYNC();
    SGX_THREADS_BEGIN(tid)
    for (int k = tid; k < cap; k += NT) cur_match[(size_t)f * cap + k] = k < Nc ? owner[k] : -1;
    if (tid == 0) nmatches_out[f] = s_total;
    SGX_THREADS_END
}

SGX_KERNEL(256) k_make_map_points(int cap, int half, const uint8_t *keys_raw, const int *n, const float *xw, const uint8_t *has, const uint8_t *desc,
                                  const float *Tcw, SgxScales sc, int nlevels, float *m_xw, float *m_normal, float *m_min, float *m_max, uint8_t *m_desc, uint8_t *m_skip)
{
    SGX_THREADS_BEGIN(tid)
    const int f = (int)blockIdx.y, i = (int)blockIdx.x * 256 + tid;
    if (i < cap) {
        const size_t o = (size_t)f * cap + i, m = (size_t)f * 2 * cap + (size_t)half * cap + i;
        const bool ok = i < n[f] && has[o];
        m_skip[m] = ok ? 0 : 1;
        if (ok) {
            const float *T = Tcw + 16 * f;
            float P[3], PO[3];
            for (int r = 0; r < 3; r++) {
                double s = 0; for (int k = 0; k < 3; k++) s += (double)T[4 * k + r] * (double)T[4 * k + 3];
                P[r] = xw[3 * o + r]; PO[r] = P[r] - (float)(s * -1.0);
            }
            const double nrm = sqrt((double)PO[0] * PO[0] + (double)PO[1] * PO[1] + (double)PO[2] * PO[2]);
            const float dist = (float)nrm, inv = (float)(1.0 / nrm);
            const int oct = ((const int *)(keys_raw + o * 28))[5];
            const float mx = dist * sc.s[oct];
            for (int r = 0; r < 3; r++) { m_xw[3 * m + r] = P[r]; m_normal[3 * m + r] = PO[r] * inv; }
            m_max[m] = mx; m_min[m] = mx / sc.s[nlevels - 1];
            const uint32_t *d = (const uint32_t *)(desc + o * 32); uint32_t *dd = (uint32_t *)(m_desc + m * 32);
#pragma unroll
            for (int w = 0; w < 8; w++) dd[w] = d[w];
        }
    }
    SGX_THREADS_END
}

SGX_KERNEL(256) k_merge_matches(int cap, const int *n, const int *match_last, const uint8_t *outlier_last, const int *match_local, int *merged, int *cur_mp_obs)
{
    SGX_THREADS_BEGIN(tid)
    const int f = (int)blockIdx.y, i = (int)blockIdx.x * 256 + tid;
    if (i < cap) {
        const size_t o = (size_t)f * cap + i;
        int idx = -1;
        if (i < n[f]) {
            if (match_local && match_local[o] >= 0) idx = cap + match_local[o];
            else if (match_last[o] >= 0 && !outlier_last[o]) idx = match_last[o];
        }
        if (merged) merged[o] = idx;
        if (cur_mp_obs) cur_mp_obs[o] = (i < n[f] && match_last[o] >= 0 && !outlier_last[o]) ? 0 : -1;
    }
    SGX_THREADS_END
}

SGX_KERNEL(256) k_gather_xw(int cap, const float *xw_last, const float *m_xw, float *xw_all)
{
    SGX_THREADS_BEGIN(tid)
    const int f = (int)blockIdx.y, i = (int)blockIdx.x * 256 + tid;
    if (i < 3 * cap) {
        const float *src = i < cap ? xw_last + 3 * ((size_t)f * cap + i) : m_xw + 3 * ((size_t)f * 2 * cap + (i - cap));
        float *dst = xw_all + 3 * ((size_t)f * 3 * cap + i);
        dst[0] = src[0]; dst[1] = src[1]; dst[2] = src[2];
    }
    SGX_THREADS_END
}

SGX_KERNEL(64) k_gray_from_color(int W, int H, const uint8_t *src, int src_pitch, int channels, int blue_first, uint8_t *dst, int dst_pitch)
{
    SGX_THREADS_BEGIN(tid)
    const int x4 = ((int)blockIdx.x * 64 + tid) * 4, y = (int)blockIdx.y, b = (int)blockIdx.z;
    if (x4 < W) {
        const uint8_t *row = src + ((size_t)b * H + y) * src_pitch + (size_t)x4 * channels;
        uint32_t out = 0;
        const int c0 = blue_first ? 1868 : 4899, c2 = blue_first ? 4899 : 1868;
        uint32_t w[4];
        const int nd = channels;
        for (int i = 0; i < 4; i++) w[i] = (i < nd && x4 + 4 <= W) ? ((const uint32_t *)row)[i] : 0u;
#pragma unroll
        for (int i = 0; i < 4; i++) {
            if (x4 + i < W) {
                int p0, p1, p2;
                if (x4 + 4 <= W) {
                    const int o = i * channels;
                    p0 = (w[o >> 2] >> (8 * (o & 3))) & 255; p1 = (w[(o + 1) >> 2] >> (8 * ((o + 1) & 3))) & 255; p2 = (w[(o + 2) >> 2] >> (8 * ((o + 2) & 3))) & 255;
                } else { p0 = row[i * channels]; p1 = row[i * channels + 1]; p2 = row[i * channels + 2]; }
                const int v = (p0 * c0 + p1 * 9617 + p2 * c2 + (1 << 13)) >> 14;
                out |= (uint32_t)v << (8 * i);
            }
        }
        uint8_t *d = dst + ((size_t)b * H + y) * dst_pitch + x4;
        if (x4 + 4 <= W) *(uint32_t *)d = out;
        else for (int i = 0; x4 + i < W; i++) d[i] = (uint8_t)(out >> (8 * i));
    }
    SGX_THREADS_END
}

SGX_KERNEL(256) k_flow_affine(int cap, const uint8_t *keys_raw, const int *n, const float *A, const float *shift, const float *boxes, int max_boxes, float *prev_xy)
{
    SGX_THREADS_BEGIN(tid)
    const int f = (int)blockIdx.y, i = (int)blockIdx.x * 256 + tid;
    if (i < cap) {
        const float *kp = (const float *)(keys_raw + ((size_t)f * cap + i) * 28);
        const float x = kp[0], y = kp[1];
        const float *a = A + 6 * f;
        float px = a[0] * x + a[1] * y + a[2], py = a[3] * x + a[4] * y + a[5];
        if (shift && boxes) {
            const float *bx = boxes + 4 * (size_t)f * max_boxes;
            if (x > bx[0] && x < bx[0] + bx[2] && y > bx[1] && y < bx[1] + bx[3]) { px += shift[2 * f]; py += shift[2 * f + 1]; }
        }
        prev_xy[2 * ((size_t)f * cap + i)] = px; prev_xy[2 * ((size_t)f * cap + i) + 1] = py;
    }
    SGX_THREADS_END
}
```

Measured before the change: 30860.

## Restructure projection matchers around carved dynamic LDS and templated slot counts

Measured after the change: 31070 (median of 6 runs). Within noise of the previous version (+0.7%).

```diff
diff --git a/include/sgx_debug.h b/include/sgx_debug.h
--- a/include/sgx_debug.h
+++ b/include/sgx_debug.h
@@ -41,6 +41,9 @@
 int sgx_tracker_debug_fail_after(int n);
 int sgx_debug_devmem_fail_after(int n);
 int sgx_stereo_debug_read(sgx_stereo *h, int frame, int32_t *best_idx, int32_t *best_dist, int32_t *exit_code, int32_t *best_inc, int32_t *sads);
+int sgx_debug_match_lds(int which, int cap, int mcap, int32_t info[4]);
+int sgx_debug_match_rescans(int *count);
+int sgx_debug_match_phases(int which, uint64_t stamps[10]);
 
 #ifdef __cplusplus
 }
diff --git a/sg_slam_amd/capi.py b/sg_slam_amd/capi.py
--- a/sg_slam_amd/capi.py
+++ b/sg_slam_amd/capi.py
@@ -143,7 +143,7 @@
     'sgx_det_debug_set_block_fusion', 'sgx_det_debug_set_irb', 'sgx_det_debug_set_gemm', 'sgx_det_debug_time_ops', 'sgx_det_debug_run_step', 'sgx_flow_debug_read_level',
     'sgx_flow_debug_level_size', 'sgx_flow_debug_read_slot', 'sgx_debug_corun_bf16', 'sgx_pnp_debug_betas', 'sgx_obj3d_debug_read',
     'sgx_tracker_debug_set_describe_early', 'sgx_tracker_debug_set_boxes', 'sgx_tracker_debug_sync_trace', 'sgx_tracker_debug_fail_after',
-    'sgx_debug_devmem_fail_after', 'sgx_cloud_debug_read', 'sgx_stereo_debug_read',
+    'sgx_debug_devmem_fail_after', 'sgx_cloud_debug_read', 'sgx_stereo_debug_read', 'sgx_debug_match_phases', 'sgx_debug_match_lds', 'sgx_debug_match_rescans',
 ]
 
 
diff --git a/sg_slam_amd/csrc/sgx_block.h b/sg_slam_amd/csrc/sgx_block.h
--- a/sg_slam_amd/csrc/sgx_block.h
+++ b/sg_slam_amd/csrc/sgx_block.h
@@ -12,17 +12,21 @@
 #else
 SGX_DEV void sgx_block_exclusive_scan_i32(int *a, int n, int *total, int tid)
 {
-    if (tid >= 64) return;
-    int carry = 0;
-    for (int base = 0; base < n; base += 64) {
-        const int i = base + tid;
-        const int v = i < n ? a[i] : 0;
-        int inc = v;
+    __shared__ int wave_total[16];
+    const int NT = (int)blockDim.x, per = (n + NT - 1) / NT;
+    const int lo = min(tid * per, n), hi = min(lo + per, n);
+    int sum = 0;
+    for (int i = lo; i < hi; i++) sum += a[i];
+    const int lane = tid & 63, wave = tid >> 6;
+    int inc = sum;
 #pragma unroll
-        for (int o = 1; o < 64; o <<= 1) { const int t = __shfl_up(inc, o, 64); if (tid >= o) inc += t; }
-        if (i < n) a[i] = carry + inc - v;
-        carry += __shfl(inc, 63, 64);
-    }
-    if (tid == 0) *total = carry;
+    for (int o = 1; o < 64; o <<= 1) { const int t = __shfl_up(inc, o, 64); if (lane >= o) inc += t; }
+    if (lane == 63 || tid == NT - 1) wave_total[wave] = inc;
+    __syncthreads();
+    int run = inc - sum;
+    for (int w = 0; w < wave; w++) run += wave_total[w];
+    for (int i = lo; i < hi; i++) { const int v = a[i]; a[i] = run; run += v; }
+    if (tid == NT - 1) *total = run;
+    __syncthreads();
 }
 #endif
diff --git a/sg_slam_amd/csrc/sgx_match.cpp b/sg_slam_amd/csrc/sgx_match.cpp
--- a/sg_slam_amd/csrc/sgx_match.cpp
+++ b/sg_slam_amd/csrc/sgx_match.cpp
@@ -11,6 +11,27 @@
 #include <string.h>
 #include <vector>
 
+#define SGX_MATCH_FRAME_SLOTS_MAX ((SGX_MATCH_CAP + SGX_MATCH_THREADS - 1) / SGX_MATCH_THREADS)
+static_assert(SGX_MATCH_FRAME_SLOTS_MAX <= 3 && SGX_LOCAL_CAP <= 8 * SGX_MATCH_THREADS && SGX_MATCH_THREADS % SGX_MATCH_GROUP == 0, "projection matchers: slots per thread");
+static int local_threads(int mcap) { return mcap > 4 * SGX_MATCH_THREADS ? 2 * SGX_MATCH_THREADS : SGX_MATCH_THREADS; }
+static int local_slots(int mcap) { int s = 1; while (s * local_threads(mcap) < mcap) s *= 2; return s; }
+static int match_allow_lds()
+{
+#ifndef SGX_EMU
+    static const int rc = [] {
+        const int fmax = (int)sgx_match_carve(SGX_MATCH_CAP, SGX_MATCH_CAP).total, lmax = (int)sgx_match_carve(SGX_MATCH_CAP, SGX_LOCAL_CAP).total;
+        const void *fk[] = { (const void *)k_match_project_frame<1>, (const void *)k_match_project_frame<2>, (const void *)k_match_project_frame<3> };
+        const void *lk[] = { (const void *)k_match_project_local<1, SGX_MATCH_THREADS>, (const void *)k_match_project_local<2, SGX_MATCH_THREADS>,
+                             (const void *)k_match_project_local<4, SGX_MATCH_THREADS>, (const void *)k_match_project_local<4, 2 * SGX_MATCH_THREADS> };
+        for (const void *k : fk) if (hipFuncSetAttribute(k, hipFuncAttributeMaxDynamicSharedMemorySize, fmax) != hipSuccess) return (int)SGX_ERR_DEVICE;
+        for (const void *k : lk) if (hipFuncSetAttribute(k, hipFuncAttributeMaxDynamicSharedMemorySize, lmax) != hipSuccess) return (int)SGX_ERR_DEVICE;
+        return (int)SGX_OK;
+    }();
+    return rc;
+#else
+    return SGX_OK;
+#endif
+}
 
 extern "C" int sgx_match_project_frame_batch_dev(
     int batch, int cap,
@@ -24,11 +45,18 @@
     if (!d_ckeys || !d_cdesc || !d_curight || !d_cn || !d_cTcw || !d_lkeys || !d_ln || !d_l_has_mp || !d_l_outlier || !d_l_xw ||
         !d_l_obs || !d_l_mpdesc || !d_lTcw || !d_cur_match || !d_nmatches) return SGX_ERR_INVALID;
     const SgxScales sc = to_scales(scale_factors, nlevels);
+    if (match_allow_lds() != SGX_OK) return SGX_ERR_DEVICE;
+    const SgxMatchCarve cv = sgx_match_carve(cap, cap);
     sgx_prof_begin(SGX_K_MATCH, (sgx_stream_t)stream);
-    static const int mthreads = sgx_getenv("SGX_TUNE_MATCH_THREADS") ? atoi(sgx_getenv("SGX_TUNE_MATCH_THREADS")) : SGX_MATCH_THREADS;
-    SGX_LAUNCH(k_match_project_frame, dim3(batch), dim3(mthreads), (sgx_stream_t)stream, cap,
-               (const uint8_t *)d_ckeys, d_cdesc, d_curight, d_cn, d_cTcw, (const uint8_t *)d_lkeys, d_ln, d_l_has_mp, d_l_outlier,
-               d_l_xw, d_l_obs, d_l_mpdesc, d_lTcw, to_cam(cam), sc, th, b_mono, check_orientation, d_cur_match, d_nmatches);
+#define SGX_FRAME_LAUNCH(S_) SGX_LAUNCH_DYN(k_match_project_frame<S_>, dim3(batch), dim3(SGX_MATCH_THREADS), cv.total, (sgx_stream_t)stream, cv, cap, \
+               (const uint8_t *)d_ckeys, d_cdesc, d_curight, d_cn, d_cTcw, (const uint8_t *)d_lkeys, d_ln, d_l_has_mp, d_l_outlier, \
+               d_l_xw, d_l_obs, d_l_mpdesc, d_lTcw, to_cam(cam), sc, th, b_mono, check_orientation, d_cur_match, d_nmatches)
+    switch ((cap + SGX_MATCH_THREADS - 1) / SGX_MATCH_THREADS) {
+    case 1: SGX_FRAME_LAUNCH(1); break;
+    case 2: SGX_FRAME_LAUNCH(2); break;
+    default: SGX_FRAME_LAUNCH(3); break;
+    }
+#undef SGX_FRAME_LAUNCH
     sgx_prof_end(SGX_K_MATCH, (sgx_stream_t)stream);
     SGX_CHECK_HIP(hipGetLastError());
     return SGX_OK;
@@ -71,10 +99,19 @@
     if (!d_ckeys || !d_cdesc || !d_curight || !d_cn || !d_cTcw || !d_mn || !d_m_xw || !d_m_normal || !d_m_min_dist || !d_m_max_dist || !d_m_desc || !d_m_obs ||
         !d_m_skip || !d_cur_match || !d_nmatches || !d_in_view) return SGX_ERR_INVALID;
     const SgxScales sc = to_scales(scale_factors, nlevels);
+    if (match_allow_lds() != SGX_OK) return SGX_ERR_DEVICE;
+    const SgxMatchCarve cv = sgx_match_carve(cap, mcap);
     sgx_prof_begin(SGX_K_MATCH_LOCAL, (sgx_stream_t)stream);
-    SGX_LAUNCH(k_match_project_local, dim3(batch), dim3(SGX_MATCH_THREADS), (sgx_stream_t)stream, cap, (const uint8_t *)d_ckeys, d_cdesc, d_curight, d_cn, d_cTcw,
-               d_cur_mp_obs, mcap, d_mn, d_m_xw, d_m_normal, d_m_min_dist, d_m_max_dist, d_m_desc, d_m_obs, d_m_skip, to_cam(cam), sc, nlevels, log_scale_factor,
-               th, nnratio, viewing_cos_limit, d_cur_match, d_nmatches, d_in_view);
+#define SGX_LOCAL_LAUNCH(S_, T_) SGX_LAUNCH_DYN((k_match_project_local<S_, T_>), dim3(batch), dim3(T_), cv.total, (sgx_stream_t)stream, cv, cap, (const uint8_t *)d_ckeys, \
+               d_cdesc, d_curight, d_cn, d_cTcw, d_cur_mp_obs, mcap, d_mn, d_m_xw, d_m_normal, d_m_min_dist, d_m_max_dist, d_m_desc, d_m_obs, d_m_skip, to_cam(cam), sc, nlevels, \
+               log_scale_factor, th, nnratio, viewing_cos_limit, d_cur_match, d_nmatches, d_in_view)
+    if (local_threads(mcap) != SGX_MATCH_THREADS) SGX_LOCAL_LAUNCH(4, 2 * SGX_MATCH_THREADS);
+    else switch (local_slots(mcap)) {
+    case 1: SGX_LOCAL_LAUNCH(1, SGX_MATCH_THREADS); break;
+    case 2: SGX_LOCAL_LAUNCH(2, SGX_MATCH_THREADS); break;
+    default: SGX_LOCAL_LAUNCH(4, SGX_MATCH_THREADS); break;
+    }
+#undef SGX_LOCAL_LAUNCH
     sgx_prof_end(SGX_K_MATCH_LOCAL, (sgx_stream_t)stream);
     SGX_CHECK_HIP(hipGetLastError());
     return SGX_OK;
@@ -202,3 +239,43 @@
     SGX_CHECK_HIP(hipGetLastError());
     return SGX_OK;
 }
+
+SGX_TAP int sgx_debug_match_lds(int which, int cap, int mcap, int32_t info[4])
+{
+    if (which < 0 || which > 1 || cap < 1 || cap > SGX_MATCH_CAP || !info || (which == 1 && (mcap < 1 || mcap > SGX_LOCAL_CAP))) return SGX_ERR_INVALID;
+    info[0] = (int32_t)sgx_match_carve(cap, which ? mcap : cap).total;
+    info[1] = which ? local_threads(mcap) : SGX_MATCH_THREADS;
+    info[2] = which ? local_slots(mcap) : (cap + SGX_MATCH_THREADS - 1) / SGX_MATCH_THREADS;
+    info[3] = SGX_MATCH_GROUP;
+    return SGX_OK;
+}
+
+SGX_TAP int sgx_debug_match_rescans(int *count)
+{
+    if (!count) return SGX_ERR_INVALID;
+    *count = 0;
+#ifdef SGX_DEBUG_TAPS
+#ifdef SGX_EMU
+    *count = g_match_rescans; g_match_rescans = 0;
+#else
+    const int zero = 0;
+    SGX_CHECK_HIP(hipDeviceSynchronize());
+    SGX_CHECK_HIP(hipMemcpyFromSymbol(count, HIP_SYMBOL(g_match_rescans), sizeof(int)));
+    SGX_CHECK_HIP(hipMemcpyToSymbol(HIP_SYMBOL(g_match_rescans), &zero, sizeof(int)));
+#endif
+#endif
+    return SGX_OK;
+}
+
+SGX_TAP int sgx_debug_match_phases(int which, uint64_t stamps[10])
+{
+    if (which < 0 || which > 1 || !stamps) return SGX_ERR_INVALID;
+    memset(stamps, 0, 10 * sizeof(uint64_t));
+#if defined(SGX_DEBUG_TAPS) && !defined(SGX_EMU)
+    unsigned long long all[2][10];
+    SGX_CHECK_HIP(hipDeviceSynchronize());
+    SGX_CHECK_HIP(hipMemcpyFromSymbol(all, HIP_SYMBOL(g_match_stamp), sizeof all));
+    for (int i = 0; i < 10; i++) stamps[i] = all[which][i];
+#endif
+    return SGX_OK;
+}
diff --git a/sg_slam_amd/csrc/sgx_match_kernels.h b/sg_slam_amd/csrc/sgx_match_kernels.h
--- a/sg_slam_amd/csrc/sgx_match_kernels.h
+++ b/sg_slam_amd/csrc/sgx_match_kernels.h
@@ -4,154 +4,409 @@
 #define SGX_GRID_COLS 64
 #define SGX_GRID_ROWS 48
 #define SGX_MATCH_CAP 1280
-#define SGX_MATCH_THREADS 1024
+#define SGX_MATCH_THREADS 512
 
 #include "sgx_match_common.h"
 
-
-SGX_KERNEL(SGX_MATCH_THREADS) k_match_project_frame(
-    int cap, const uint8_t *ckeys_raw, const uint8_t *cdesc, const float *curight, const int *cn, const float *cTcw,
+#if defined(SGX_DEBUG_TAPS) && !defined(SGX_EMU)
+static __device__ unsigned long long g_match_stamp[2][10];
+#define SGX_MATCH_STAMP(which, slot) do { if (blockIdx.x == 0 && threadIdx.x == 0) g_match_stamp[which][slot] = wall_clock64(); } while (0)
+#define SGX_MATCH_STAMP_VAL(which, slot, v) do { if (blockIdx.x == 0 && threadIdx.x == 0) g_match_stamp[which][slot] = (unsigned long long)(v); } while (0)
+#else
+#define SGX_MATCH_STAMP(which, slot) ((void)0)
+#define SGX_MATCH_STAMP_VAL(which, slot, v) ((void)0)
+#endif
+
+#define SGX_GRID_CELLS (SGX_GRID_COLS * SGX_GRID_ROWS)
+#ifndef SGX_EMU
+SGX_DEV float sgx_uniform_f32(float x) { return __int_as_float(__builtin_amdgcn_readfirstlane(__float_as_int(x))); }
+#else
+SGX_DEV float sgx_uniform_f32(float x) { return x; }
+#endif
+#define SGX_MATCH_KEEP 4
+#ifndef SGX_MATCH_GROUP
+#define SGX_MATCH_GROUP 4
+#endif
+#define SGX_MATCH_WAVES_PER_SIMD (2 * SGX_MATCH_THREADS / 256)
+
+struct __attribute__((aligned(16))) SgxKeyRec { float x, y, ur; uint32_t info; };
+struct __attribute__((aligned(16))) SgxDesc8 { uint32_t w[8]; };
+
+struct SgxMatchCarve { uint32_t rec, desc, lock_a, lock_b, owner, choice, cell_start, cell_list, misc, total; };
+
+static inline SgxMatchCarve sgx_match_carve(int cap, int npts)
+{
+    const uint32_t c4 = ((uint32_t)cap + 3u) & ~3u, locks = 12u * c4, counters = 4u * SGX_GRID_CELLS;
+    SgxMatchCarve c; uint32_t o = 0;
+    c.rec = o; o += 16u * c4;
+    c.desc = o; o += 32u * c4;
+    c.lock_a = o; c.lock_b = o + 4u * c4; c.owner = o + 8u * c4; o += locks > counters ? locks : counters;
+    c.choice = o; o = (o + 2u * (uint32_t)npts + 15u) & ~15u;
+    c.cell_start = o; o = (o + 2u * (SGX_GRID_CELLS + 1) + 15u) & ~15u;
+    c.cell_list = o; o = (o + 2u * c4 + 15u) & ~15u;
+    c.misc = o; o += 4u * 72u;
+    c.total = o;
+    return c;
+}
+
+struct SgxMatchLds { SgxKeyRec *rec; SgxDesc8 *desc; int *lock_a, *lock_b, *owner, *cnt, *misc; uint16_t *choice, *cell_start, *cell_list; };
+enum { SGX_MS_CHANGED = 0 , SGX_MS_TOTAL = 2, SGX_MS_REJECTED = 3, SGX_MS_NGRID = 4, SGX_MS_HIST = 8, SGX_MS_BAD = 8 + SGX_HISTO };
+
+SGX_DEV SgxMatchLds sgx_match_lds(unsigned char *pool, const SgxMatchCarve &c)
+{
+    SgxMatchLds L;
+    L.rec = (SgxKeyRec *)(pool + c.rec); L.desc = (SgxDesc8 *)(pool + c.desc);
+    L.lock_a = (int *)(pool + c.lock_a); L.lock_b = (int *)(pool + c.lock_b); L.owner = (int *)(pool + c.owner); L.cnt = (int *)(pool + c.lock_a);
+    L.misc = (int *)(pool + c.misc);
+    L.choice = (uint16_t *)(pool + c.choice); L.cell_start = (uint16_t *)(pool + c.cell_start); L.cell_list = (uint16_t *)(pool + c.cell_list);
+    return L;
+}
+
+#ifdef SGX_DEBUG_TAPS
+#ifdef SGX_EMU
+static int g_match_rescans;
+#else
+static __device__ int g_match_rescans;
+#endif
+#define SGX_MATCH_COUNT_RESCAN() sgx_atomic_add(&g_match_rescans, 1)
+#else
+#define SGX_MATCH_COUNT_RESCAN() ((void)0)
+#endif
+
+#define SGX_LKEY(dd, px, py, k) (((uint32_t)(dd) << 23) | ((uint32_t)(px) << 17) | ((uint32_t)(py) << 11) | (uint32_t)(k))
+#define SGX_LKEY_NONE 0xFFFFFFFFu
+
+SGX_DEV void sgx_match_stage_grid(const SgxMatchLds &L, int which, int f, int cap, int Nc, const uint8_t *ckeys_raw, const uint8_t *cdesc, const float *curight,
+                                  const int *cur_mp_obs, const SgxCam &cam, float invW, float invH)
+{
+    const int NT = (int)blockDim.x;
+    SGX_THREADS_BEGIN(tid)
+    for (int k = tid; k < Nc; k += NT) {
+        const float *kp = (const float *)(ckeys_raw + ((size_t)f * cap + k) * 28);
+        const float x = kp[0], y = kp[1];
+        const int oct = ((const int *)kp)[5];
+        const int px = (int)round((double)((x - cam.minX) * invW)), py = (int)round((double)((y - cam.minY) * invH));
+        const bool valid = !(px < 0 || px >= SGX_GRID_COLS || py < 0 || py >= SGX_GRID_ROWS);
+        const bool held = cur_mp_obs && cur_mp_obs[(size_t)f * cap + k] > 0;
+        SgxKeyRec r; r.x = x; r.y = y; r.ur = curight[(size_t)f * cap + k];
+        r.info = (uint32_t)(oct & 0xFF) | ((uint32_t)(px & 0xFF) << 8) | ((uint32_t)(py & 0xFF) << 16) | (held ? 0x40000000u : 0u) | (valid ? 0x80000000u : 0u);
+        L.rec[k] = r;
+        const uint32_t *d = (const uint32_t *)(cdesc + ((size_t)f * cap + k) * 32);
+        SgxDesc8 dd;
+#pragma unroll
+        for (int w = 0; w < 8; w++) dd.w[w] = d[w];
+        L.desc[k] = dd;
+    }
+    for (int i = tid; i < SGX_GRID_CELLS; i += NT) L.cnt[i] = 0;
+    SGX_THREADS_END
+    SGX_SYNC();
+    SGX_MATCH_STAMP(which, 1);
+    SGX_THREADS_BEGIN(tid)
+    for (int k = tid; k < Nc; k += NT) { const uint32_t inf = L.rec[k].info; if (inf & 0x80000000u) sgx_atomic_add(&L.cnt[((inf >> 8) & 0xFF) * SGX_GRID_ROWS + ((inf >> 16) & 0xFF)], 1); }
+    SGX_THREADS_END
+    SGX_SYNC();
+    SGX_MATCH_STAMP(which, 2);
+    SGX_THREADS_BEGIN(tid)
+    sgx_block_exclusive_scan_i32(L.cnt, SGX_GRID_CELLS, &L.misc[SGX_MS_NGRID], tid);
+    SGX_THREADS_END
+    SGX_SYNC();
+    SGX_MATCH_STAMP(which, 3);
+    SGX_THREADS_BEGIN(tid)
+    for (int k = tid; k < Nc; k += NT) {
+        const uint32_t inf = L.rec[k].info;
+        if (inf & 0x80000000u) L.cell_list[sgx_atomic_add(&L.cnt[((inf >> 8) & 0xFF) * SGX_GRID_ROWS + ((inf >> 16) & 0xFF)], 1)] = (uint16_t)k;
+    }
+    SGX_THREADS_END
+    SGX_SYNC();
+    SGX_THREADS_BEGIN(tid)
+    for (int i = tid; i < SGX_GRID_CELLS; i += NT) L.cell_start[i + 1] = (uint16_t)L.cnt[i];
+    if (tid == 0) L.cell_start[0] = 0;
+    SGX_THREADS_END
+    SGX_SYNC();
+    SGX_MATCH_STAMP(which, 4);
+}
+
+struct SgxWin { float u, v, radius, ur; int minLevel, maxLevel, c0x, c1x, c0y, c1y; bool chk; };
+
+SGX_DEV bool sgx_win_cells(SgxWin &w, const SgxCam &cam, float invW, float invH)
+{
+    w.c0x = max(0, (int)floorf((w.u - cam.minX - w.radius) * invW)); w.c1x = min(SGX_GRID_COLS - 1, (int)ceilf((w.u - cam.minX + w.radius) * invW));
+    w.c0y = max(0, (int)floorf((w.v - cam.minY - w.radius) * invH)); w.c1y = min(SGX_GRID_ROWS - 1, (int)ceilf((w.v - cam.minY + w.radius) * invH));
+    return !(w.c0x >= SGX_GRID_COLS || w.c1x < 0 || w.c0y >= SGX_GRID_ROWS || w.c1y < 0);
+}
+
+template <bool LOCKED, class Visit>
+SGX_DEV void sgx_window_walk(const SgxMatchLds &L, const SgxWin &w, const uint32_t *dm, const int *lock, int i, int first, int step, Visit visit)
+{
+    for (int px = w.c0x; px <= w.c1x; px++)
+    for (int q = L.cell_start[px * SGX_GRID_ROWS + w.c0y] + first, qe = L.cell_start[px * SGX_GRID_ROWS + w.c1y + 1]; q < qe; q += step) {
+        const int k = L.cell_list[q];
+        const SgxKeyRec r = L.rec[k];
+        const int oct = r.info & 0xFF, py = (r.info >> 16) & 0xFF;
+        if (w.chk) { if (oct < w.minLevel) continue; if (w.maxLevel >= 0 && oct > w.maxLevel) continue; }
+        if (!(fabsf(r.x - w.u) < w.radius && fabsf(r.y - w.v) < w.radius)) continue;
+        if (LOCKED) { if (lock[k] < i) continue; }
+        if (r.ur > 0) { if (fabsf(w.ur - r.ur) > w.radius) continue; }
+        const SgxDesc8 d = L.desc[k];
+        visit(SGX_LKEY(sgx_hamming256(dm, d.w), px, py, k));
+    }
+}
+
+SGX_DEV void sgx_keep_insert(uint32_t &c0, uint32_t &c1, uint32_t &c2, uint32_t &c3, uint32_t key)
+{
+    if (key < c3) {
+        c3 = key;
+        if (c3 < c2) { const uint32_t t = c2; c2 = c3; c3 = t; }
+        if (c2 < c1) { const uint32_t t = c1; c1 = c2; c2 = t; }
+        if (c1 < c0) { const uint32_t t = c0; c0 = c1; c1 = t; }
+    }
+}
+
+SGX_DEV int sgx_match_point(int tid, int s, int NT) { return tid / SGX_MATCH_GROUP + (s * SGX_MATCH_GROUP + (tid & (SGX_MATCH_GROUP - 1))) * (NT / SGX_MATCH_GROUP); }
+
+#ifndef SGX_EMU
+template <int CTRL> SGX_DEV uint32_t sgx_dpp(uint32_t v) { return (uint32_t)__builtin_amdgcn_update_dpp((int)v, (int)v, CTRL, 0xF, 0xF, false); }
+SGX_DEV uint32_t sgx_group_min(uint32_t v)
+{
+    v = min(v, sgx_dpp<0xB1>(v)); v = min(v, sgx_dpp<0x4E>(v));
+    if (SGX_MATCH_GROUP >= 8) v = min(v, sgx_dpp<0x141>(v));
+    if (SGX_MATCH_GROUP >= 16) v = min(v, sgx_dpp<0x140>(v));
+    return v;
+}
+SGX_DEV uint32_t sgx_group_sum(uint32_t v)
+{
+    v += sgx_dpp<0xB1>(v); v += sgx_dpp<0x4E>(v);
+    if (SGX_MATCH_GROUP >= 8) v += sgx_dpp<0x141>(v);
+    if (SGX_MATCH_GROUP >= 16) v += sgx_dpp<0x140>(v);
+    return v;
+}
+#endif
+
+template <int SLOTS, class Proj>
+SGX_DEV void sgx_match_build(const SgxMatchLds &L, int N, int tid, int NT, const uint8_t *descs, uint32_t *ckey, uint32_t *cflag, Proj proj)
+{
+#ifdef SGX_EMU
+    uint32_t flags = 0;
+    for (int s = 0; s < SLOTS; s++) {
+        const int i = sgx_match_point(tid, s, NT);
+        uint32_t c0 = SGX_LKEY_NONE, c1 = SGX_LKEY_NONE, c2 = SGX_LKEY_NONE, c3 = SGX_LKEY_NONE, fl = 0;
+        if (i < N) {
+            SgxWin w;
+            if (proj(i, w, fl)) {
+                const uint32_t *dmp = (const uint32_t *)(descs + (size_t)i * 32);
+                uint32_t dm[8]; for (int q = 0; q < 8; q++) dm[q] = dmp[q];
+                int cnt = 0;
+                sgx_window_walk<false>(L, w, dm, nullptr, 0, 0, 1, [&](uint32_t key) { cnt++; sgx_keep_insert(c0, c1, c2, c3, key); });
+                if (cnt > SGX_MATCH_KEEP) fl |= 1u;
+            }
+        }
+        ckey[s * SGX_MATCH_KEEP + 0] = c0; ckey[s * SGX_MATCH_KEEP + 1] = c1; ckey[s * SGX_MATCH_KEEP + 2] = c2; ckey[s * SGX_MATCH_KEEP + 3] = c3;
+        flags |= fl << (2 * s);
+    }
+    cflag[0] = flags;
+#else
+    const int lane = tid & (SGX_MATCH_GROUP - 1), g = tid / SGX_MATCH_GROUP, NG = NT / SGX_MATCH_GROUP;
+#pragma unroll
+    for (int q = 0; q < SLOTS * SGX_MATCH_KEEP; q++) ckey[q] = SGX_LKEY_NONE;
+    uint32_t flags = 0;
+#pragma unroll 1
+    for (int s = 0; s < SLOTS; s++) {
+        float w_u = 0.f, w_v = 0.f, w_r = 0.f, w_ur = 0.f; uint32_t w_cells = 0, w_gate = 0;
+        {
+            const int i = g + (s * SGX_MATCH_GROUP + lane) * NG;
+            SgxWin w; uint32_t fl = 0;
+            const bool ok = i < N && proj(i, w, fl);
+            if (ok) {
+                w_u = w.u; w_v = w.v; w_r = w.radius; w_ur = w.ur;
+                w_cells = (uint32_t)w.c0x | ((uint32_t)w.c1x << 6) | ((uint32_t)w.c0y << 12) | ((uint32_t)w.c1y << 18) | (1u << 24);
+            }
+            w_gate = (uint32_t)((w.minLevel + 1) & 0xFF) | ((uint32_t)((w.maxLevel + 1) & 0xFF) << 8) | (w.chk ? 1u << 16 : 0u) | (fl << 17);
+            if (!ok) w_gate &= 3u << 17;
+        }
+        uint32_t dnext[8] = { 0, 0, 0, 0, 0, 0, 0, 0 };
+        if (SLOTS < 4 && g + s * SGX_MATCH_GROUP * NG < N) {
+            const uint32_t *dmp = (const uint32_t *)(descs + (size_t)(g + s * SGX_MATCH_GROUP * NG) * 32);
+#pragma unroll
+            for (int q = 0; q < 8; q++) dnext[q] = dmp[q];
+        }
+#pragma unroll 1
+        for (int jj = 0; jj < SGX_MATCH_GROUP; jj++) {
+            const int i = g + (s * SGX_MATCH_GROUP + jj) * NG;
+            SgxWin w;
+            w.u = __shfl(w_u, jj, SGX_MATCH_GROUP); w.v = __shfl(w_v, jj, SGX_MATCH_GROUP); w.radius = __shfl(w_r, jj, SGX_MATCH_GROUP); w.ur = __shfl(w_ur, jj, SGX_MATCH_GROUP);
+            const uint32_t cells = (uint32_t)__shfl((int)w_cells, jj, SGX_MATCH_GROUP), gate = (uint32_t)__shfl((int)w_gate, jj, SGX_MATCH_GROUP);
+            w.c0x = cells & 63; w.c1x = (cells >> 6) & 63; w.c0y = (cells >> 12) & 63; w.c1y = (cells >> 18) & 63;
+            w.minLevel = (int)(gate & 0xFF) - 1; w.maxLevel = (int)((gate >> 8) & 0xFF) - 1; w.chk = (gate >> 16) & 1u;
+            uint32_t fl = (gate >> 17) & 3u;
+            uint32_t c0 = SGX_LKEY_NONE, c1 = SGX_LKEY_NONE, c2 = SGX_LKEY_NONE, c3 = SGX_LKEY_NONE, cnt = 0;
+            uint32_t dm[8] = { 0, 0, 0, 0, 0, 0, 0, 0 };
+            if (SLOTS < 4) {
+#pragma unroll
+                for (int q = 0; q < 8; q++) dm[q] = dnext[q];
+                if (jj + 1 < SGX_MATCH_GROUP && i + NG < N) {
+                    const uint32_t *dmp = (const uint32_t *)(descs + (size_t)(i + NG) * 32);
+#pragma unroll
+                    for (int q = 0; q < 8; q++) dnext[q] = dmp[q];
+                }
+            } else if (cells >> 24) {
+                const uint32_t *dmp = (const uint32_t *)(descs + (size_t)i * 32);
+#pragma unroll
+                for (int q = 0; q < 8; q++) dm[q] = dmp[q];
+            }
+            if (cells >> 24)
+                sgx_window_walk<false>(L, w, dm, nullptr, 0, lane, SGX_MATCH_GROUP, [&](uint32_t key) { cnt++; sgx_keep_insert(c0, c1, c2, c3, key); });
+            cnt = sgx_group_sum(cnt);
+            uint32_t o[SGX_MATCH_KEEP];
+#pragma unroll
+            for (int q = 0; q < SGX_MATCH_KEEP; q++) {
+                const uint32_t m = sgx_group_min(c0);
+                if (c0 == m) { c0 = c1; c1 = c2; c2 = c3; c3 = SGX_LKEY_NONE; }
+                o[q] = m;
+            }
+            if (cnt > (uint32_t)SGX_MATCH_KEEP) fl |= 1u;
+            if (lane == jj) flags |= fl << (2 * s);
+#pragma unroll
+            for (int t = 0; t < SLOTS; t++)
+                if (lane == jj && t == s) {
+#pragma unroll
+                    for (int q = 0; q < SGX_MATCH_KEEP; q++) ckey[t * SGX_MATCH_KEEP + q] = o[q];
+                }
+        }
+    }
+    cflag[0] = flags;
+#endif
+}
+
+struct SgxFrameProj { float Rcw[3][3], tcw[3]; bool bForward, bBackward; };
+
+SGX_DEV bool sgx_frame_window(size_t li, const uint8_t *l_has_mp, const uint8_t *l_outlier, const float *l_xw, const uint8_t *lkeys_raw, const SgxFrameProj &P,
+                              const SgxCam &cam, const SgxScales &sc, float th, float invW, float invH, SgxWin &w)
+{
+    if (!(l_has_mp[li] && !l_outlier[li])) return false;
+    const float *xw = l_xw + 3 * li;
+    const float x3x = sgx_gemm3(P.Rcw[0], xw, P.tcw[0]), x3y = sgx_gemm3(P.Rcw[1], xw, P.tcw[1]), x3z = sgx_gemm3(P.Rcw[2], xw, P.tcw[2]);
+    const float invzc = (float)(1.0 / (double)x3z);
+    const float u = cam.fx * x3x * invzc + cam.cx, v = cam.fy * x3y * invzc + cam.cy;
+    if (!(!(invzc < 0) && !(u < cam.minX || u > cam.maxX) && !(v < cam.minY || v > cam.maxY))) return false;
+    const int lo = ((const int *)(lkeys_raw + li * 28))[5];
+    w.u = u; w.v = v; w.radius = th * sc.s[lo];
+    if (P.bForward) { w.minLevel = lo; w.maxLevel = -1; } else if (P.bBackward) { w.minLevel = 0; w.maxLevel = lo; } else { w.minLevel = lo - 1; w.maxLevel = lo + 1; }
+    w.chk = (w.minLevel > 0) || (w.maxLevel >= 0);
+    w.ur = u - cam.bf * invzc;
+    return sgx_win_cells(w, cam, invW, invH);
+}
+
+template <int SLOTS>
+SGX_KERNEL_OCC(SGX_MATCH_THREADS, SGX_MATCH_WAVES_PER_SIMD) k_match_project_frame(
+    SgxMatchCarve cv, int cap, const uint8_t *ckeys_raw, const uint8_t *cdesc, const float *curight, const int *cn, const float *cTcw,
     const uint8_t *lkeys_raw, const int *ln, const uint8_t *l_has_mp, const uint8_t *l_outlier, const float *l_xw,
     const int *l_obs, const uint8_t *l_mpdesc, const float *lTcw,
     SgxCam cam, SgxScales sc, float th, int bMono, int check_ori, int *cur_match, int *nmatches_out)
 {
-    SGX_LDS float kx[SGX_MATCH_CAP], ky[SGX_MATCH_CAP], kur[SGX_MATCH_CAP], kang[SGX_MATCH_CAP];
-    SGX_LDS uint32_t kinfo[SGX_MATCH_CAP];
-    SGX_LDS uint32_t kdesc[SGX_MATCH_CAP * 8];
-    SGX_LDS int lock_a[SGX_MATCH_CAP], lock_b[SGX_MATCH_CAP];
-    SGX_LDS int choice[SGX_MATCH_CAP];
-    SGX_LDS int owner[SGX_MATCH_CAP];
-    SGX_LDS int hist[SGX_HISTO], bad[SGX_HISTO];
-    SGX_LDS int cell_start[SGX_GRID_COLS * SGX_GRID_ROWS + 1];
-    SGX_LDS int cell_fill[SGX_GRID_COLS * SGX_GRID_ROWS];
-    SGX_LDS uint16_t cell_list[SGX_MATCH_CAP];
-    SGX_LDS int s_changed, s_total, s_rejected, s_ngrid;
+    SGX_DYN_LDS(pool);
+    const SgxMatchLds L = sgx_match_lds(pool, cv);
+    int *hist = L.misc + SGX_MS_HIST, *bad = L.misc + SGX_MS_BAD;
+    SGX_PRIV_DECL(uint32_t, ckey, SLOTS * SGX_MATCH_KEEP, SGX_MATCH_THREADS);
+    SGX_PRIV_DECL(uint32_t, cflag, 1, SGX_MATCH_THREADS);
 
     const int f = (int)blockIdx.x;
+    SGX_MATCH_STAMP(0, 0);
     SGX_WAVE_PRIORITY(3);
     const int Nc = min(cn[f], cap), Nl = min(ln[f], cap);
     const int NT = (int)blockDim.x;
     const float *Tc = cTcw + 16 * f, *Tl = lTcw + 16 * f;
-    const float invW = (float)SGX_GRID_COLS / (cam.maxX - cam.minX), invH = (float)SGX_GRID_ROWS / (cam.maxY - cam.minY);
-
-    SGX_THREADS_BEGIN(tid)
-    for (int k = tid; k < Nc; k += NT) {
-        const float *kp = (const float *)(ckeys_raw + ((size_t)f * cap + k) * 28);
-        const float x = kp[0], y = kp[1];
-        kx[k] = x; ky[k] = y; kang[k] = kp[3]; kur[k] = curight[(size_t)f * cap + k];
-        const int oct = ((const int *)kp)[5];
-        const int px = (int)round((double)((x - cam.minX) * invW)), py = (int)round((double)((y - cam.minY) * invH));
-        const bool valid = !(px < 0 || px >= SGX_GRID_COLS || py < 0 || py >= SGX_GRID_ROWS);
-        kinfo[k] = (uint32_t)(oct & 0xFF) | ((uint32_t)(px & 0xFF) << 8) | ((uint32_t)(py & 0xFF) << 16) | (valid ? 0x80000000u : 0u);
-        const uint32_t *d = (const uint32_t *)(cdesc + ((size_t)f * cap + k) * 32);
-#pragma unroll
-        for (int w = 0; w < 8; w++) kdesc[k * 8 + w] = d[w];
-        lock_a[k] = 0x7FFFFFFF; owner[k] = -1;
-    }
-    for (int i = tid; i < SGX_HISTO; i += NT) { hist[i] = 0; bad[i] = 0; }
-    for (int i = tid; i < SGX_GRID_COLS * SGX_GRID_ROWS; i += NT) { cell_start[i] = 0; cell_fill[i] = 0; }
-    if (tid == 0) { s_total = 0; s_rejected = 0; }
-    SGX_THREADS_END
-    SGX_SYNC();
-    SGX_THREADS_BEGIN(tid)
-    for (int k = tid; k < Nc; k += NT) { const uint32_t inf = kinfo[k]; if (inf & 0x80000000u) sgx_atomic_add(&cell_start[((inf >> 8) & 0xFF) * SGX_GRID_ROWS + ((inf >> 16) & 0xFF)], 1); }
-    SGX_THREADS_END
-    SGX_SYNC();
-    SGX_THREADS_BEGIN(tid)
-    sgx_block_exclusive_scan_i32(cell_start, SGX_GRID_COLS * SGX_GRID_ROWS, &s_ngrid, tid);
-    SGX_THREADS_END
-    SGX_SYNC();
-    SGX_THREADS_BEGIN(tid)
-    if (tid == 0) cell_start[SGX_GRID_COLS * SGX_GRID_ROWS] = s_ngrid;
-    for (int k = tid; k < Nc; k += NT) {
-        const uint32_t inf = kinfo[k];
-        if (inf & 0x80000000u) { const int c = ((inf >> 8) & 0xFF) * SGX_GRID_ROWS + ((inf >> 16) & 0xFF); cell_list[cell_start[c] + sgx_atomic_add(&cell_fill[c], 1)] = (uint16_t)k; }
-    }
-    SGX_THREADS_END
-    SGX_SYNC();
-
-    float Rcw[3][3], tcw[3];
-    for (int r = 0; r < 3; r++) { for (int c = 0; c < 3; c++) Rcw[r][c] = Tc[4 * r + c]; tcw[r] = Tc[4 * r + 3]; }
+    const float invW = sgx_uniform_f32((float)SGX_GRID_COLS / (cam.maxX - cam.minX)), invH = sgx_uniform_f32((float)SGX_GRID_ROWS / (cam.maxY - cam.minY));
+
+    sgx_match_stage_grid(L, 0, f, cap, Nc, ckeys_raw, cdesc, curight, nullptr, cam, invW, invH);
+
+    SgxFrameProj P;
+    for (int r = 0; r < 3; r++) { for (int c = 0; c < 3; c++) P.Rcw[r][c] = Tc[4 * r + c]; P.tcw[r] = Tc[4 * r + 3]; }
     float twc[3];
     for (int i = 0; i < 3; i++) {
-        double s = 0; for (int k = 0; k < 3; k++) s += (double)Rcw[k][i] * (double)tcw[k];
+        double s = 0; for (int k = 0; k < 3; k++) s += (double)P.Rcw[k][i] * (double)P.tcw[k];
         twc[i] = (float)(s * -1.0);
     }
     const float Rl2[3] = { Tl[8], Tl[9], Tl[10] };
     const float tlc2 = sgx_gemm3(Rl2, twc, Tl[11]);
     const float mb = cam.bf / cam.fx;
-    const bool bForward = tlc2 > mb && !bMono, bBackward = -tlc2 > mb && !bMono;
-
-    int *lock_cur = lock_a, *lock_new = lock_b;
+    P.bForward = tlc2 > mb && !bMono; P.bBackward = -tlc2 > mb && !bMono;
+
+    SGX_THREADS_BEGIN(tid)
+    SGX_PRIV_BIND(ckey, tid); SGX_PRIV_BIND(cflag, tid);
+    for (int k = tid; k < Nc; k += NT) { L.lock_a[k] = 0x7FFFFFFF; L.lock_b[k] = 0x7FFFFFFF; L.owner[k] = -1; }
+    for (int i = tid; i < SGX_HISTO; i += NT) { hist[i] = 0; bad[i] = 0; }
+    if (tid == 0) { L.misc[SGX_MS_CHANGED] = 0; L.misc[SGX_MS_CHANGED + 1] = 0; L.misc[SGX_MS_TOTAL] = 0; L.misc[SGX_MS_REJECTED] = 0; }
+    sgx_match_build<SLOTS>(L, Nl, tid, NT, l_mpdesc + (size_t)f * cap * 32, ckey, cflag, [&](int i, SgxWin &w, uint32_t &fl) {
+        const size_t li = (size_t)f * cap + i;
+        w.minLevel = 0; w.maxLevel = 0; w.chk = false;
+        if (!sgx_frame_window(li, l_has_mp, l_outlier, l_xw, lkeys_raw, P, cam, sc, th, invW, invH, w)) return false;
+        if (l_obs[li] > 0) fl |= 2u;
+        return true;
+    });
+    SGX_THREADS_END
+    SGX_SYNC();
+    SGX_MATCH_STAMP(0, 5);
+
+    int *lock_cur = L.lock_a, *lock_new = L.lock_b;
+    int nsweeps = 0;
     for (int sweep = 0; sweep < SGX_MATCH_CAP + 2; sweep++) {
         SGX_THREADS_BEGIN(tid)
-        if (tid == 0) s_changed = 0;
-        for (int k = tid; k < Nc; k += NT) lock_new[k] = 0x7FFFFFFF;
+        SGX_PRIV_BIND(ckey, tid); SGX_PRIV_BIND(cflag, tid);
+#pragma unroll 1
+        for (int s = 0; s < SLOTS; s++) {
+            const int i = sgx_match_point(tid, s, NT);
+            uint32_t kk[SGX_MATCH_KEEP] = { SGX_LKEY_NONE, SGX_LKEY_NONE, SGX_LKEY_NONE, SGX_LKEY_NONE };
+            const uint32_t fl = (cflag[0] >> (2 * s)) & 3u;
+#pragma unroll
+            for (int t = 0; t < SLOTS; t++) if (t == s) {
+#pragma unroll
+                for (int q = 0; q < SGX_MATCH_KEEP; q++) kk[q] = ckey[t * SGX_MATCH_KEEP + q];
+            }
+            if (i < Nl) {
+                uint32_t k1 = SGX_LKEY_NONE;
+#pragma unroll
+                for (int q = 0; q < SGX_MATCH_KEEP; q++) {
+                    const uint32_t key = kk[q];
+                    if (k1 == SGX_LKEY_NONE && key != SGX_LKEY_NONE && !(lock_cur[key & 0x7FF] < i)) k1 = key;
+                }
+                if ((fl & 1u) && k1 == SGX_LKEY_NONE) {
+                    SGX_MATCH_COUNT_RESCAN();
+                    const size_t li = (size_t)f * cap + i;
+                    SgxWin w;
+                    if (sgx_frame_window(li, l_has_mp, l_outlier, l_xw, lkeys_raw, P, cam, sc, th, invW, invH, w)) {
+                        uint32_t dm[8];
+#pragma unroll
+                        for (int q = 0; q < 8; q++) dm[q] = ((const uint32_t *)(l_mpdesc + li * 32))[q];
+                        sgx_window_walk<true>(L, w, dm, lock_cur, i, 0, 1, [&](uint32_t key) { k1 = key < k1 ? key : k1; });
+                    }
+                }
+                const int best = (k1 != SGX_LKEY_NONE && (int)(k1 >> 23) <= SGX_TH_HIGH) ? (int)(k1 & 0x7FF) : -1;
+                L.choice[i] = best >= 0 ? (uint16_t)best : (uint16_t)0xFFFF;
+                if (best >= 0 && (fl & 2u)) sgx_atomic_min_i32(&lock_new[best], i);
+            }
+        }
         SGX_THREADS_END
         SGX_SYNC();
         SGX_THREADS_BEGIN(tid)
-        for (int i = tid; i < Nl; i += NT) {
-            int best = -1;
-            const size_t li = (size_t)f * cap + i;
-            if (l_has_mp[li] && !l_outlier[li]) {
-                const float *xw = l_xw + 3 * li;
-                const float x3x = sgx_gemm3(Rcw[0], xw, tcw[0]), x3y = sgx_gemm3(Rcw[1], xw, tcw[1]), x3z = sgx_gemm3(Rcw[2], xw, tcw[2]);
-                const float invzc = (float)(1.0 / (double)x3z);
-                const float u = cam.fx * x3x * invzc + cam.cx, v = cam.fy * x3y * invzc + cam.cy;
-                if (!(invzc < 0) && !(u < cam.minX || u > cam.maxX) && !(v < cam.minY || v > cam.maxY)) {
-                    const int lo = ((const int *)(lkeys_raw + li * 28))[5];
-                    const float radius = th * sc.s[lo];
-                    int minLevel, maxLevel;
-                    if (bForward) { minLevel = lo; maxLevel = -1; } else if (bBackward) { minLevel = 0; maxLevel = lo; } else { minLevel = lo - 1; maxLevel = lo + 1; }
-                    const int c0x = max(0, (int)floorf((u - cam.minX - radius) * invW)), c1x = min(SGX_GRID_COLS - 1, (int)ceilf((u - cam.minX + radius) * invW));
-                    const int c0y = max(0, (int)floorf((v - cam.minY - radius) * invH)), c1y = min(SGX_GRID_ROWS - 1, (int)ceilf((v - cam.minY + radius) * invH));
-                    if (!(c0x >= SGX_GRID_COLS || c1x < 0 || c0y >= SGX_GRID_ROWS || c1y < 0)) {
-                        const bool chk = (minLevel > 0) || (maxLevel >= 0);
-                        const float ur = u - cam.bf * invzc;
-                        const uint32_t *dmp = (const uint32_t *)(l_mpdesc + li * 32);
-                        uint32_t dm[8];
-#pragma unroll
-                        for (int w = 0; w < 8; w++) dm[w] = dmp[w];
-                        unsigned long long bestKey = ~0ull;
-                        for (int px = c0x; px <= c1x; px++)
-                        for (int q = cell_start[px * SGX_GRID_ROWS + c0y], qe = cell_start[px * SGX_GRID_ROWS + c1y + 1]; q < qe; q++) {
-                            const int k = cell_list[q];
-                            const uint32_t inf = kinfo[k];
-                            const int oct = inf & 0xFF, py = (inf >> 16) & 0xFF;
-                            if (chk) { if (oct < minLevel) continue; if (maxLevel >= 0 && oct > maxLevel) continue; }
-                            if (!(fabsf(kx[k] - u) < radius && fabsf(ky[k] - v) < radius)) continue;
-                            if (lock_cur[k] < i) continue;
-                            if (kur[k] > 0) { if (fabsf(ur - kur[k]) > radius) continue; }
-                            const int dist = sgx_hamming256(dm, &kdesc[k * 8]);
-                            const unsigned long long key = ((unsigned long long)dist << 28) | ((unsigned long long)px << 22) | ((unsigned long long)py << 16) | (unsigned long long)k;
-                            if (key < bestKey) bestKey = key;
-                        }
-                        if (bestKey != ~0ull && (int)(bestKey >> 28) <= SGX_TH_HIGH) best = (int)(bestKey & 0xFFFF);
-                    }
-                }
-            }
-            choice[i] = best;
-            if (best >= 0 && l_obs[li] > 0) sgx_atomic_min_i32(&lock_new[best], i);
-        }
-        SGX_THREADS_END
-        SGX_SYNC();
-        SGX_THREADS_BEGIN(tid)
-        for (int k = tid; k < Nc; k += NT) if (lock_new[k] != lock_cur[k]) s_changed = 1;
+        if (tid == 0) L.misc[SGX_MS_CHANGED + ((sweep + 1) & 1)] = 0;
+        for (int k = tid; k < Nc; k += NT) { if (lock_new[k] != lock_cur[k]) L.misc[SGX_MS_CHANGED + (sweep & 1)] = 1; lock_cur[k] = 0x7FFFFFFF; }
         SGX_THREADS_END
         SGX_SYNC();
         int *t = lock_cur; lock_cur = lock_new; lock_new = t;
-        if (!s_changed) break;
-    }
+        nsweeps++;
+        if (!L.misc[SGX_MS_CHANGED + (sweep & 1)]) break;
+    }
+    SGX_MATCH_STAMP(0, 6); SGX_MATCH_STAMP_VAL(0, 8, nsweeps);
 
     SGX_THREADS_BEGIN(tid)
     for (int i = tid; i < Nl; i += NT) {
-        const int k = choice[i];
-        if (k < 0) continue;
-        sgx_atomic_max(&owner[k], i);
-        sgx_atomic_add(&s_total, 1);
+        const int k = L.choice[i];
+        if (k == 0xFFFF) continue;
+        sgx_atomic_max(&L.owner[k], i);
+        sgx_atomic_add(&L.misc[SGX_MS_TOTAL], 1);
         if (check_ori) {
-            const float la = ((const float *)(lkeys_raw + ((size_t)f * cap + i) * 28))[3];
-            float rot = la - kang[k];
+            const float la = ((const float *)(lkeys_raw + ((size_t)f * cap + i) * 28))[3], ca = ((const float *)(ckeys_raw + ((size_t)f * cap + k) * 28))[3];
+            float rot = la - ca;
             if (rot < 0.0f) rot += 360.0f;
             int bin = (int)round((double)(rot * (SGX_HISTO / 360.0f)));
             if (bin == SGX_HISTO) bin = 0;
@@ -179,17 +434,18 @@
         SGX_SYNC();
         SGX_THREADS_BEGIN(tid)
         for (int i = tid; i < Nl; i += NT) {
-            const int k = choice[i];
-            if (k >= 0 && bad[lock_new[i]]) { sgx_atomic_add(&s_rejected, 1); lock_cur[k] = -2; }
+            const int k = L.choice[i];
+            if (k != 0xFFFF && bad[lock_new[i]]) { sgx_atomic_add(&L.misc[SGX_MS_REJECTED], 1); lock_cur[k] = -2; }
         }
         SGX_THREADS_END
         SGX_SYNC();
     }
     SGX_THREADS_BEGIN(tid)
-    for (int k = tid; k < Nc; k += NT) cur_match[(size_t)f * cap + k] = (check_ori && lock_cur[k] == -2) ? -1 : owner[k];
+    for (int k = tid; k < Nc; k += NT) cur_match[(size_t)f * cap + k] = (check_ori && lock_cur[k] == -2) ? -1 : L.owner[k];
     for (int k = Nc + tid; k < cap; k += NT) cur_match[(size_t)f * cap + k] = -1;
-    if (tid == 0) nmatches_out[f] = s_total - s_rejected;
-    SGX_THREADS_END
+    if (tid == 0) nmatches_out[f] = L.misc[SGX_MS_TOTAL] - L.misc[SGX_MS_REJECTED];
+    SGX_THREADS_END
+    SGX_MATCH_STAMP(0, 7);
 }
 
 SGX_KERNEL(256) k_stereo_from_rgbd(int cap, const uint8_t *keys_raw, const int *n, const uint16_t *depth, int W, int H,
@@ -273,8 +529,6 @@
 }
 
 #define SGX_LOCAL_CAP 4096
-#define SGX_LOCAL_SLOTS (SGX_LOCAL_CAP / SGX_MATCH_THREADS)
-#define SGX_LOCAL_KEEP 4
 
 struct SgxLocalProj { float u, v, radius, projXR; int lvl; bool ok; };
 
@@ -306,201 +560,133 @@
     return r;
 }
 
-#define SGX_LKEY(dd, px, py, k) (((uint32_t)(dd) << 23) | ((uint32_t)(px) << 17) | ((uint32_t)(py) << 11) | (uint32_t)(k))
-#define SGX_LKEY_NONE 0xFFFFFFFFu
-
-SGX_KERNEL(SGX_MATCH_THREADS) k_match_project_local(
-    int cap, const uint8_t *ckeys_raw, const uint8_t *cdesc, const float *curight, const int *cn, const float *cTcw, const int *cur_mp_obs,
+template <int SLOTS, int THREADS>
+SGX_KERNEL_OCC(THREADS, SGX_MATCH_WAVES_PER_SIMD) k_match_project_local(
+    SgxMatchCarve cv, int cap, const uint8_t *ckeys_raw, const uint8_t *cdesc, const float *curight, const int *cn, const float *cTcw, const int *cur_mp_obs,
     int mcap, const int *mn, const float *m_xw, const float *m_normal, const float *m_min_dist, const float *m_max_dist, const uint8_t *m_desc,
     const int *m_obs, const uint8_t *m_skip,
     SgxCam cam, SgxScales sc, int nlevels, float log_scale_factor, float th, float nnratio, float viewing_cos_limit,
     int *cur_match, int *nmatches_out, uint8_t *in_view)
 {
-    SGX_LDS float kx[SGX_MATCH_CAP], ky[SGX_MATCH_CAP], kur[SGX_MATCH_CAP];
-    SGX_LDS uint32_t kinfo[SGX_MATCH_CAP];
-    SGX_LDS uint32_t kdesc[SGX_MATCH_CAP * 8];
-    SGX_LDS int lock_a[SGX_MATCH_CAP], lock_b[SGX_MATCH_CAP];
-    SGX_LDS int owner[SGX_MATCH_CAP];
-    SGX_LDS int cell_start[SGX_GRID_COLS * SGX_GRID_ROWS + 1];
-    SGX_LDS int cell_fill[SGX_GRID_COLS * SGX_GRID_ROWS];
-    SGX_LDS uint16_t cell_list[SGX_MATCH_CAP];
-    SGX_LDS uint16_t choice[SGX_LOCAL_CAP];
-    SGX_LDS int s_changed, s_total, s_ngrid;
-    SGX_PRIV_DECL(uint32_t, ckey, SGX_LOCAL_SLOTS * SGX_LOCAL_KEEP, SGX_MATCH_THREADS);
-    SGX_PRIV_DECL(uint32_t, cflag, SGX_LOCAL_SLOTS, SGX_MATCH_THREADS);
+    SGX_DYN_LDS(pool);
+    const SgxMatchLds L = sgx_match_lds(pool, cv);
+    SGX_PRIV_DECL(uint32_t, ckey, SLOTS * SGX_MATCH_KEEP, THREADS);
+    SGX_PRIV_DECL(uint32_t, cflag, 1, THREADS);
 
     const int f = (int)blockIdx.x;
+    SGX_MATCH_STAMP(1, 0);
     SGX_WAVE_PRIORITY(3);
-    const int Nc = min(cn[f], cap), Nm = min(min(mn[f], mcap), SGX_LOCAL_CAP);
     const int NT = (int)blockDim.x;
+    const int Nc = min(cn[f], cap), Nm = min(min(mn[f], mcap), SLOTS * THREADS);
     const float *Tc = cTcw + 16 * f;
-    const float invW = (float)SGX_GRID_COLS / (cam.maxX - cam.minX), invH = (float)SGX_GRID_ROWS / (cam.maxY - cam.minY);
-
-    SGX_THREADS_BEGIN(tid)
-    for (int k = tid; k < Nc; k += NT) {
-        const float *kp = (const float *)(ckeys_raw + ((size_t)f * cap + k) * 28);
-        const float x = kp[0], y = kp[1];
-        kx[k] = x; ky[k] = y; kur[k] = curight[(size_t)f * cap + k];
-        const int oct = ((const int *)kp)[5];
-        const int px = (int)round((double)((x - cam.minX) * invW)), py = (int)round((double)((y - cam.minY) * invH));
-        const bool valid = !(px < 0 || px >= SGX_GRID_COLS || py < 0 || py >= SGX_GRID_ROWS);
-        kinfo[k] = (uint32_t)(oct & 0xFF) | ((uint32_t)(px & 0xFF) << 8) | ((uint32_t)(py & 0xFF) << 16) | (valid ? 0x80000000u : 0u);
-        const uint32_t *d = (const uint32_t *)(cdesc + ((size_t)f * cap + k) * 32);
-#pragma unroll
-        for (int w = 0; w < 8; w++) kdesc[k * 8 + w] = d[w];
-        lock_a[k] = (cur_mp_obs && cur_mp_obs[(size_t)f * cap + k] > 0) ? -1 : 0x7FFFFFFF;
-        owner[k] = -1;
-    }
-    for (int i = tid; i < SGX_GRID_COLS * SGX_GRID_ROWS; i += NT) { cell_start[i] = 0; cell_fill[i] = 0; }
-    if (tid == 0) s_total = 0;
-    SGX_THREADS_END
-    SGX_SYNC();
-    SGX_THREADS_BEGIN(tid)
-    for (int k = tid; k < Nc; k += NT) { const uint32_t inf = kinfo[k]; if (inf & 0x80000000u) sgx_atomic_add(&cell_start[((inf >> 8) & 0xFF) * SGX_GRID_ROWS + ((inf >> 16) & 0xFF)], 1); }
-    SGX_THREADS_END
-    SGX_SYNC();
-    SGX_THREADS_BEGIN(tid)
-    sgx_block_exclusive_scan_i32(cell_start, SGX_GRID_COLS * SGX_GRID_ROWS, &s_ngrid, tid);
-    SGX_THREADS_END
-    SGX_SYNC();
-    SGX_THREADS_BEGIN(tid)
-    if (tid == 0) cell_start[SGX_GRID_COLS * SGX_GRID_ROWS] = s_ngrid;
-    for (int k = tid; k < Nc; k += NT) {
-        const uint32_t inf = kinfo[k];
-        if (inf & 0x80000000u) { const int c = ((inf >> 8) & 0xFF) * SGX_GRID_ROWS + ((inf >> 16) & 0xFF); cell_list[cell_start[c] + sgx_atomic_add(&cell_fill[c], 1)] = (uint16_t)k; }
-    }
-    SGX_THREADS_END
-    SGX_SYNC();
+    const float invW = sgx_uniform_f32((float)SGX_GRID_COLS / (cam.maxX - cam.minX)), invH = sgx_uniform_f32((float)SGX_GRID_ROWS / (cam.maxY - cam.minY));
+
+    sgx_match_stage_grid(L, 1, f, cap, Nc, ckeys_raw, cdesc, curight, cur_mp_obs, cam, invW, invH);
 
     float Rcw[3][3], tcw[3], Ow[3];
     for (int r = 0; r < 3; r++) { for (int c = 0; c < 3; c++) Rcw[r][c] = Tc[4 * r + c]; tcw[r] = Tc[4 * r + 3]; }
-    for (int i = 0; i < 3; i++) { double s = 0; for (int k = 0; k < 3; k++) s += (double)Rcw[k][i] * (double)tcw[k]; Ow[i] = (float)(s * -1.0); }
+    for (int i = 0; i < 3; i++) { double s = 0; for (int k = 0; k < 3; k++) s += (double)Rcw[k][i] * (double)tcw[k]; Ow[i] = sgx_uniform_f32((float)(s * -1.0)); }
+
+    auto window = [&](size_t mi, SgxWin &w) {
+        const SgxLocalProj pr = sgx_local_project(m_xw + 3 * mi, m_normal + 3 * mi, m_max_dist[mi], m_min_dist[mi], Rcw, tcw, Ow, cam, sc, nlevels,
+                                                  log_scale_factor, th, viewing_cos_limit);
+        w.u = pr.u; w.v = pr.v; w.radius = pr.radius; w.ur = pr.projXR; w.minLevel = pr.lvl - 1; w.maxLevel = pr.lvl; w.chk = true;
+        return pr.ok;
+    };
 
     SGX_THREADS_BEGIN(tid)
     SGX_PRIV_BIND(ckey, tid); SGX_PRIV_BIND(cflag, tid);
-#pragma unroll
-    for (int j = 0; j < SGX_LOCAL_SLOTS; j++) {
-        const int i = tid + j * SGX_MATCH_THREADS;
-        uint32_t c0 = SGX_LKEY_NONE, c1 = SGX_LKEY_NONE, c2 = SGX_LKEY_NONE, c3 = SGX_LKEY_NONE, flag = 0;
-        if (i < Nm) {
-            const size_t mi = (size_t)f * mcap + i;
-            uint8_t vis = 0;
-            if (!m_skip[mi]) {
-                const SgxLocalProj pr = sgx_local_project(m_xw + 3 * mi, m_normal + 3 * mi, m_max_dist[mi], m_min_dist[mi], Rcw, tcw, Ow, cam, sc, nlevels,
-                                                          log_scale_factor, th, viewing_cos_limit);
-                if (pr.ok) {
-                    vis = 1;
-                    if (m_obs[mi] > 0) flag |= 2u;
-                    const float u = pr.u, v = pr.v, radius = pr.radius;
-                    const int minLevel = pr.lvl - 1, maxLevel = pr.lvl;
-                    const int c0x = max(0, (int)floorf((u - cam.minX - radius) * invW)), c1x = min(SGX_GRID_COLS - 1, (int)ceilf((u - cam.minX + radius) * invW));
-                    const int c0y = max(0, (int)floorf((v - cam.minY - radius) * invH)), c1y = min(SGX_GRID_ROWS - 1, (int)ceilf((v - cam.minY + radius) * invH));
-                    if (!(c0x >= SGX_GRID_COLS || c1x < 0 || c0y >= SGX_GRID_ROWS || c1y < 0)) {
-                        const uint32_t *dmp = (const uint32_t *)(m_desc + mi * 32);
-                        uint32_t dm[8];
-#pragma unroll
-                        for (int w = 0; w < 8; w++) dm[w] = dmp[w];
-                        int cnt = 0;
-                        for (int px = c0x; px <= c1x; px++)
-                        for (int q = cell_start[px * SGX_GRID_ROWS + c0y], qe = cell_start[px * SGX_GRID_ROWS + c1y + 1]; q < qe; q++) {
-                            const int k = cell_list[q];
-                            const uint32_t inf = kinfo[k];
-                            const int oct = inf & 0xFF, py = (inf >> 16) & 0xFF;
-                            if (oct < minLevel || oct > maxLevel) continue;
-                            if (!(fabsf(kx[k] - u) < radius && fabsf(ky[k] - v) < radius)) continue;
-                            if (kur[k] > 0) { if (fabsf(pr.projXR - kur[k]) > radius) continue; }
-                            const int dd = sgx_hamming256(dm, &kdesc[k * 8]);
-                            uint32_t key = SGX_LKEY(dd, px, py, k);
-                            cnt++;
-                            if (key < c3) {
-                                c3 = key;
-                                if (c3 < c2) { const uint32_t t = c2; c2 = c3; c3 = t; }
-                                if (c2 < c1) { const uint32_t t = c1; c1 = c2; c2 = t; }
-                                if (c1 < c0) { const uint32_t t = c0; c0 = c1; c1 = t; }
-                            }
-                        }
-                        if (cnt > SGX_LOCAL_KEEP) flag |= 1u;
-                    }
-                }
-            }
-            in_view[mi] = vis;
-        }
-        ckey[j * SGX_LOCAL_KEEP + 0] = c0; ckey[j * SGX_LOCAL_KEEP + 1] = c1; ckey[j * SGX_LOCAL_KEEP + 2] = c2; ckey[j * SGX_LOCAL_KEEP + 3] = c3;
-        cflag[j] = flag;
-    }
-    SGX_THREADS_END
-    SGX_SYNC();
-
-    int *lock_cur = lock_a, *lock_new = lock_b;
+    for (int k = tid; k < Nc; k += NT) { const int l0 = (L.rec[k].info & 0x40000000u) ? -1 : 0x7FFFFFFF; L.lock_a[k] = l0; L.lock_b[k] = l0; L.owner[k] = -1; }
+    if (tid == 0) { L.misc[SGX_MS_CHANGED] = 0; L.misc[SGX_MS_CHANGED + 1] = 0; L.misc[SGX_MS_TOTAL] = 0; }
+    sgx_match_build<SLOTS>(L, Nm, tid, NT, m_desc + (size_t)f * mcap * 32, ckey, cflag, [&](int i, SgxWin &w, uint32_t &fl) {
+        const size_t mi = (size_t)f * mcap + i;
+        bool ok = false;
+        w.minLevel = 0; w.maxLevel = 0; w.chk = true;
+        if (!m_skip[mi]) ok = window(mi, w);
+        in_view[mi] = ok ? 1 : 0;
+        if (!ok) return false;
+        if (m_obs[mi] > 0) fl |= 2u;
+        return sgx_win_cells(w, cam, invW, invH);
+    });
+    SGX_THREADS_END
+    SGX_SYNC();
+    SGX_MATCH_STAMP(1, 5);
+
+    int *lock_cur = L.lock_a, *lock_new = L.lock_b;
+    int nsweeps = 0;
     for (int sweep = 0; sweep < SGX_LOCAL_CAP + 2; sweep++) {
         SGX_THREADS_BEGIN(tid)
-        if (tid == 0) s_changed = 0;
-        for (int k = tid; k < Nc; k += NT) lock_new[k] = (cur_mp_obs && cur_mp_obs[(size_t)f * cap + k] > 0) ? -1 : 0x7FFFFFFF;
+        SGX_PRIV_BIND(ckey, tid); SGX_PRIV_BIND(cflag, tid);
+#pragma unroll 1
+        for (int s = 0; s < SLOTS; s++) {
+            const int i = sgx_match_point(tid, s, NT);
+            uint32_t kk[SGX_MATCH_KEEP] = { SGX_LKEY_NONE, SGX_LKEY_NONE, SGX_LKEY_NONE, SGX_LKEY_NONE };
+            const uint32_t fl = (cflag[0] >> (2 * s)) & 3u;
+#pragma unroll
+            for (int t = 0; t < SLOTS; t++) if (t == s) {
+#pragma unroll
+                for (int q = 0; q < SGX_MATCH_KEEP; q++) kk[q] = ckey[t * SGX_MATCH_KEEP + q];
+            }
+            if (i < Nm) {
+                uint32_t k1 = SGX_LKEY_NONE, k2 = SGX_LKEY_NONE;
+#pragma unroll
+                for (int q = 0; q < SGX_MATCH_KEEP; q++) {
+                    const uint32_t key = kk[q];
+                    const bool avail = key != SGX_LKEY_NONE && !(lock_cur[key & 0x7FF] < i), first = avail && k1 == SGX_LKEY_NONE, second = avail && !first && k2 == SGX_LKEY_NONE;
+                    k1 = first ? key : k1; k2 = second ? key : k2;
+                }
+                bool rescan = (fl & 1u) && k2 == SGX_LKEY_NONE;
+                if (rescan && k1 != SGX_LKEY_NONE) {
+                    const int d1 = (int)(k1 >> 23), d4 = (int)(kk[SGX_MATCH_KEEP - 1] >> 23);
+                    if (d1 > SGX_TH_HIGH || (nnratio >= 0.0f && !((float)d1 > nnratio * (float)d4))) rescan = false;
+                }
+                if (rescan) {
+                    SGX_MATCH_COUNT_RESCAN();
+                    const size_t mi = (size_t)f * mcap + i;
+                    SgxWin w;
+                    window(mi, w); sgx_win_cells(w, cam, invW, invH);
+                    uint32_t r1 = SGX_LKEY_NONE, r2 = SGX_LKEY_NONE, dm[8];
+#pragma unroll
+                    for (int q = 0; q < 8; q++) dm[q] = ((const uint32_t *)(m_desc + mi * 32))[q];
+                    sgx_window_walk<true>(L, w, dm, lock_cur, i, 0, 1,
+                                          [&](uint32_t key) { const bool b1 = key < r1, b2 = key < r2; r2 = b1 ? r1 : (b2 ? key : r2); r1 = b1 ? key : r1; });
+                    k1 = r1; k2 = r2;
+                }
+                int best = -1;
+                if (k1 != SGX_LKEY_NONE) {
+                    const int bestDist = (int)(k1 >> 23), bestLevel = (int)(L.rec[k1 & 0x7FF].info & 0xFF);
+                    const int bestDist2 = k2 != SGX_LKEY_NONE ? (int)(k2 >> 23) : 256, bestLevel2 = k2 != SGX_LKEY_NONE ? (int)(L.rec[k2 & 0x7FF].info & 0xFF) : -1;
+                    if (bestDist <= SGX_TH_HIGH && !(bestLevel == bestLevel2 && (float)bestDist > nnratio * (float)bestDist2)) best = (int)(k1 & 0x7FF);
+                }
+                L.choice[i] = best >= 0 ? (uint16_t)best : (uint16_t)0xFFFF;
+                if (best >= 0 && (fl & 2u)) sgx_atomic_min_i32(&lock_new[best], i);
+            }
+        }
         SGX_THREADS_END
         SGX_SYNC();
         SGX_THREADS_BEGIN(tid)
-        SGX_PRIV_BIND(ckey, tid); SGX_PRIV_BIND(cflag, tid);
-#pragma unroll
-        for (int j = 0; j < SGX_LOCAL_SLOTS; j++) {
-            const int i = tid + j * SGX_MATCH_THREADS;
-            if (i < Nm) {
-                uint32_t k1 = SGX_LKEY_NONE, k2 = SGX_LKEY_NONE;
-#pragma unroll
-                for (int q = 0; q < SGX_LOCAL_KEEP; q++) {
-                    const uint32_t key = ckey[j * SGX_LOCAL_KEEP + q];
-                    if (key != SGX_LKEY_NONE && !(lock_cur[key & 0x7FF] < i)) { if (k1 == SGX_LKEY_NONE) k1 = key; else if (k2 == SGX_LKEY_NONE) k2 = key; }
-                }
-                if ((cflag[j] & 1u) && k2 == SGX_LKEY_NONE) {
-                    const size_t mi = (size_t)f * mcap + i;
-                    const SgxLocalProj pr = sgx_local_project(m_xw + 3 * mi, m_normal + 3 * mi, m_max_dist[mi], m_min_dist[mi], Rcw, tcw, Ow, cam, sc, nlevels,
-                                                              log_scale_factor, th, viewing_cos_limit);
-                    const float u = pr.u, v = pr.v, radius = pr.radius;
-                    const int minLevel = pr.lvl - 1, maxLevel = pr.lvl;
-                    const int c0x = max(0, (int)floorf((u - cam.minX - radius) * invW)), c1x = min(SGX_GRID_COLS - 1, (int)ceilf((u - cam.minX + radius) * invW));
-                    const int c0y = max(0, (int)floorf((v - cam.minY - radius) * invH)), c1y = min(SGX_GRID_ROWS - 1, (int)ceilf((v - cam.minY + radius) * invH));
-                    const uint32_t *dm = (const uint32_t *)(m_desc + mi * 32);
-                    k1 = SGX_LKEY_NONE; k2 = SGX_LKEY_NONE;
-                    for (int px = c0x; px <= c1x; px++)
-                    for (int q = cell_start[px * SGX_GRID_ROWS + c0y], qe = cell_start[px * SGX_GRID_ROWS + c1y + 1]; q < qe; q++) {
-                        const int k = cell_list[q];
-                        const uint32_t inf = kinfo[k];
-                        const int oct = inf & 0xFF, py = (inf >> 16) & 0xFF;
-                        if (oct < minLevel || oct > maxLevel) continue;
-                        if (!(fabsf(kx[k] - u) < radius && fabsf(ky[k] - v) < radius)) continue;
-                        if (lock_cur[k] < i) continue;
-                        if (kur[k] > 0) { if (fabsf(pr.projXR - kur[k]) > radius) continue; }
-                        const uint32_t key = SGX_LKEY(sgx_hamming256(dm, &kdesc[k * 8]), px, py, k);
-                        if (key < k1) { k2 = k1; k1 = key; } else if (key < k2) k2 = key;
-                    }
-                }
-                int best = -1;
-                if (k1 != SGX_LKEY_NONE) {
-                    const int bestDist = (int)(k1 >> 23), bestLevel = (int)(kinfo[k1 & 0x7FF] & 0xFF);
-                    const int bestDist2 = k2 != SGX_LKEY_NONE ? (int)(k2 >> 23) : 256, bestLevel2 = k2 != SGX_LKEY_NONE ? (int)(kinfo[k2 & 0x7FF] & 0xFF) : -1;
-                    if (bestDist <= SGX_TH_HIGH && !(bestLevel == bestLevel2 && (float)bestDist > nnratio * (float)bestDist2)) best = (int)(k1 & 0x7FF);
-                }
-                choice[i] = best >= 0 ? (uint16_t)best : (uint16_t)0xFFFF;
-                if (best >= 0 && (cflag[j] & 2u)) sgx_atomic_min_i32(&lock_new[best], i);
-            }
-        }
-        SGX_THREADS_END
-        SGX_SYNC();
-        SGX_THREADS_BEGIN(tid)
-        for (int k = tid; k < Nc; k += NT) if (lock_new[k] != lock_cur[k]) s_changed = 1;
+        if (tid == 0) L.misc[SGX_MS_CHANGED + ((sweep + 1) & 1)] = 0;
+        for (int k = tid; k < Nc; k += NT) {
+            if (lock_new[k] != lock_cur[k]) L.misc[SGX_MS_CHANGED + (sweep & 1)] = 1;
+            lock_cur[k] = (L.rec[k].info & 0x40000000u) ? -1 : 0x7FFFFFFF;
+        }
         SGX_THREADS_END
         SGX_SYNC();
         int *t = lock_cur; lock_cur = lock_new; lock_new = t;
-        if (!s_changed) break;
-    }
-
-    SGX_THREADS_BEGIN(tid)
-    for (int i = tid; i < Nm; i += NT) { const int k = choice[i]; if (k != 0xFFFF) { sgx_atomic_max(&owner[k], i); sgx_atomic_add(&s_total, 1); } }
-    SGX_THREADS_END
-    SGX_SYNC();
-    SGX_THREADS_BEGIN(tid)
-    for (int k = tid; k < cap; k += NT) cur_match[(size_t)f * cap + k] = k < Nc ? owner[k] : -1;
-    if (tid == 0) nmatches_out[f] = s_total;
-    SGX_THREADS_END
+        nsweeps++;
+        if (!L.misc[SGX_MS_CHANGED + (sweep & 1)]) break;
+    }
+    SGX_MATCH_STAMP(1, 6); SGX_MATCH_STAMP_VAL(1, 8, nsweeps);
+
+    SGX_THREADS_BEGIN(tid)
+    for (int i = tid; i < Nm; i += NT) { const int k = L.choice[i]; if (k != 0xFFFF) { sgx_atomic_max(&L.owner[k], i); sgx_atomic_add(&L.misc[SGX_MS_TOTAL], 1); } }
+    SGX_THREADS_END
+    SGX_SYNC();
+    SGX_THREADS_BEGIN(tid)
+    for (int k = tid; k < cap; k += NT) cur_match[(size_t)f * cap + k] = k < Nc ? L.owner[k] : -1;
+    if (tid == 0) nmatches_out[f] = L.misc[SGX_MS_TOTAL];
+    SGX_THREADS_END
+    SGX_MATCH_STAMP(1, 7);
 }
 
 SGX_KERNEL(256) k_make_map_points(int cap, int half, const uint8_t *keys_raw, const int *n, const float *xw, const uint8_t *has, const uint8_t *desc,
```
